# kevinh-e/BetaOne

Hardware: AMD Instinct MI355X
Metric: mcts_nodes_per_sec (higher is better)
Workload: dtype f32 (3 x f16 split, f32 accumulate)

## Files before the change

### betaone_amd/csrc/bo_engine.cpp

```cpp
#include "../../include/betaone_engine.h"
#include "../../include/betaone_lab.h"

#include "bo_tree.h"
#include "bo_fastw.h"
#include "bo_select_wide.h"
#include "bo_replay.h"
#include "bo_train.h"
#include "bo_metrics.h"
#include "bo_pgn.h"
#include "bo_san.h"
#include "bo_analyse.h"
#include "bo_reanalyse.h"
#include "bo_perft.h"
#include "bo_book.h"
#include "bo_merge.h"
#include "bo_tb.h"
#include "bo_nn_fused.h"
#include "bo_conv.h"
#include "bo_tower.h"
#include "bo_tower_wg.h"
#include "bo_tower_h.h"
#include "bo_tower_s.h"
#include "bo_tower_s16.h"
#include "bo_tower_h16.h"
#include "bo_heads.h"
#include "bo_tower_b1.h"
#include "bo_rt.h"
#include "bo_hostrng.h"

#include <math.h>
#include <stdio.h>
#include <string.h>
#include <string>
#include <vector>
#include <algorithm>
#include <deque>
#include <memory>
#include <type_traits>

static thread_local std::string g_err;
static int fail(int code, const std::string &msg) {
    g_err = msg;
    return code;
}
#define RT(call)                                                                                     \
    do {                                                                                             \
        int _rc = (call);                                                                            \
        if (_rc != 0) return fail(BO_E_HIP, std::string(#call) + ": " + rt_errstr(_rc));             \
    } while (0)

struct bo_engine {
    Eng d;
    FastW f;
    int fast_reuse = 1;
    int sel_profile = 0, sel_pending = 0;
    long long sel_launches = 0;
    double sel_ms = 0.0;
#if !defined(BO_WAVE_EMU)
    hipEvent_t sel_ev0 = nullptr, sel_ev1 = nullptr;
#endif
    bool fast = false;
    bo_config cfg;
    int device;
    std::vector<void *> allocs;
    int *d_go = nullptr, *d_action = nullptr;
    std::vector<int> h_i32;
    std::vector<HostRng> rng;
    int *d_res_blk = nullptr, *d_info_blk = nullptr;
    int *h_res = nullptr, *h_info = nullptr;
    int watch_seen = 0;
    double *h_noise = nullptr;
    int *h_go = nullptr;
    int *h_action = nullptr;
    int action_flip = 0;
    rt_event ev_action[2]{};
    bool ev_action_made[2] = {false, false};
    bool ship = true;
    bool prefetch_valid = false;
    std::vector<int> h_nl, h_term;
    bool nl_valid = false;
    void *setup_dev = nullptr, *setup_host = nullptr;
    size_t setup_cap = 0;
    std::vector<unsigned char> noise_pending;
    std::vector<int> lazy_want;
    bool begin_lazy = false, ev_begin_made = false;
    rt_event ev_begin{};
    double *h_turn_u = nullptr;
    int *h_turn_flags = nullptr;
    double *d_turn_pw = nullptr;
    std::vector<double> turn_pw_host;
    double turn_pw_tfinal = 0.0;
    int *d_turn_action = nullptr, *d_turn_state = nullptr, *d_turn_cres = nullptr;
    float *d_turn_rv = nullptr;
    int *d_turn_resigned = nullptr, *d_turn_rnext = nullptr;
    std::vector<int> resign_en;
    float resign_t = 0.0f;
    int resign_k = 1;
    float *d_root_value = nullptr;
    TbTable *d_tb_tabs = nullptr;
    std::vector<int> turn_want;
    bool turn_outstanding = false, ev_turn_made = false;
    rt_event ev_turn{};
    template <class T> int alloc(T **p, size_t n) {
        void *v = nullptr;
        int rc = rt_malloc(&v, n * sizeof(T));
        if (rc) return rc;
        allocs.push_back(v);
        *p = (T *)v;
        return 0;
    }
};

extern "C" int bo_abi_version(void) { return BO_ABI_VERSION; }
extern "C" const char *bo_last_error(void) { return g_err.c_str(); }

static const char *START_FEN = "rnbqkbnr/pppppppp/8/8/8/8/PPPPPPPP/RNBQKBNR w KQkq - 0 1";

static bool parse_fen(const char *fen, DPos *out) {
    memset(out, 0, sizeof(*out));
    const char *s = fen;
    while (*s == ' ') s++;
    int r = 7, f = 0;
    for (; *s && *s != ' '; s++) {
        char c = *s;
        if (c == '/') { r--; f = 0; continue; }
        if (c >= '1' && c <= '8') { f += c - '0'; continue; }
        int white = (c >= 'A' && c <= 'Z');
        char l = (char)(white ? c - 'A' + 'a' : c);
        int t = l == 'p' ? 0 : l == 'n' ? 1 : l == 'b' ? 2 : l == 'r' ? 3 : l == 'q' ? 4 : l == 'k' ? 5 : -1;
        if (t < 0 || r < 0 || f > 7) return false;
        out->bb[t] |= BIT(r * 8 + f);
        out->bb[white ? BB_WHITE : BB_BLACK] |= BIT(r * 8 + f);
        f++;
    }
    int turn = 1, ep = -1, half = 0, full = 1;
    uint32_t cr = 0;
    while (*s == ' ') s++;
    if (*s) { if (*s == 'w') turn = 1; else if (*s == 'b') turn = 0; else return false; s++; }
    while (*s == ' ') s++;
    for (; *s && *s != ' '; s++) {
        if (*s == 'K') cr |= 0x02u; else if (*s == 'Q') cr |= 0x04u; else if (*s == 'k') cr |= 0x08u;
        else if (*s == 'q') cr |= 0x10u; else if (*s != '-') return false;
    }
    const uint64_t wk = out->bb[BB_K] & out->bb[BB_WHITE] & BIT(4), bk = out->bb[BB_K] & out->bb[BB_BLACK] & BIT(60);
    const uint64_t wr = out->bb[BB_R] & out->bb[BB_WHITE], br = out->bb[BB_R] & out->bb[BB_BLACK];
    if (!wk || !(wr & BIT(7))) cr &= ~0x02u;
    if (!wk || !(wr & BIT(0))) cr &= ~0x04u;
    if (!bk || !(br & BIT(63))) cr &= ~0x08u;
    if (!bk || !(br & BIT(56))) cr &= ~0x10u;
    while (*s == ' ') s++;
    if (*s) {
        if (*s != '-') {
            if (s[0] < 'a' || s[0] > 'h' || s[1] < '1' || s[1] > '8') return false;
            ep = (s[1] - '1') * 8 + (s[0] - 'a');
            s += 2;
        } else s++;
    }
    while (*s == ' ') s++;
    if (*s) half = (int)strtol(s, (char **)&s, 10);
    while (*s == ' ') s++;
// ... 70 lines not shown
    c.nstride = c.NCAP;
    c.PLY_CAP = cfg->max_plies; c.TRK_CAP = cfg->max_plies;
    c.UL_MAX = fast ? 1 : c.B; c.CH_MAX = ch_max < 1 ? 1 : ch_max;
    c.cpuct = (float)cfg->cpuct;
    c.keep = (float)(1.0 - cfg->dirichlet_epsilon);
    c.eps = cfg->dirichlet_epsilon;
    c.use_noise = cfg->dirichlet_alpha > 0 ? 1 : 0;
    c.root_m = root_m;
    c.profile = 0;
    { const char *v = getenv("BETAONE_BURST_TWO_PATHS"); c.burst_two = (v && v[0] == '0') ? 0 : 1; }
    c.root_q = 0;
    const size_t G = (size_t)c.G, N = G * (size_t)c.NCAP;
    Eng &d = e->d;
    int rc = 0;
    float *sq = nullptr, *rcp = nullptr; int *wl = nullptr;
    rc |= e->alloc(&sq, (size_t)c.S + 2); rc |= e->alloc(&wl, (size_t)c.B + 1); rc |= e->alloc(&rcp, (size_t)c.S + 3);
    int **iscal[] = {&d.sims_done, &d.n_nodes, &d.rows, &d.n_runs, &d.n_ul, &d.req_nlegal, &d.status,
                     &d.trk_n, &d.n_hist, &d.ctx_mode, &d.root_nch, &d.stat_evals,
                     &d.stat_flushes, &d.stat_term_sims, &d.stat_levels, &d.stat_children_scanned, &e->d_go, &e->d_action};
    for (int **p : iscal) rc |= e->alloc(p, G);
    const size_t res_ints = G * (4 + 2 * (size_t)BO_RES_CAP) + 4, info_ints = G * 18;
    rc |= e->alloc(&e->d_res_blk, res_ints); rc |= e->alloc(&e->d_info_blk, info_ints);
    if (!rc) {
        d.res_n = e->d_res_blk; d.res_best_idx = e->d_res_blk + G; d.res_best_mv = e->d_res_blk + 2 * G; d.res_total = e->d_res_blk + 3 * G;
        d.res_idx = e->d_res_blk + 4 * G; d.res_val = reinterpret_cast<float *>(e->d_res_blk + 4 * G + G * BO_RES_CAP);
        d.res_watch = e->d_res_blk + G * (4 + 2 * (size_t)BO_RES_CAP); d.watch = nullptr; d.watch_n = 1;
        d.phase = e->d_info_blk; d.req_node = e->d_info_blk + G; d.root_nlegal = e->d_info_blk + 2 * G; d.root_term = e->d_info_blk + 3 * G;
        d.ply = e->d_info_blk + 4 * G;
        e->d_turn_action = e->d_info_blk + 5 * G; e->d_turn_state = e->d_info_blk + 6 * G; e->d_turn_cres = e->d_info_blk + 7 * G;
        e->d_turn_rv = reinterpret_cast<float *>(e->d_info_blk + 15 * G); e->d_turn_resigned = e->d_info_blk + 16 * G;
        e->d_turn_rnext = e->d_info_blk + 17 * G;
        rt_memset(e->d_res_blk, 0, res_ints * 4, nullptr); rt_memset(e->d_info_blk, 0, info_ints * 4, nullptr);
    }
    rc |= rt_host_alloc((void **)&e->h_res, res_ints * 4); rc |= rt_host_alloc((void **)&e->h_info, info_ints * 4);
    rc |= rt_host_alloc((void **)&e->h_noise, G * BO_MAX_MOVES * sizeof(double)); rc |= rt_host_alloc((void **)&e->h_go, G * 4);
    rc |= rt_host_alloc((void **)&e->h_action, 2 * G * 4);
    rc |= rt_host_alloc((void **)&e->h_turn_u, G * sizeof(double)); rc |= rt_host_alloc((void **)&e->h_turn_flags, G * 4);
    rc |= e->alloc(&e->d_turn_pw, (size_t)cfg->num_simulations + 1);
    { const char *v = getenv("BETAONE_TURN_COPIES"); e->ship = !(v && v[0] == '1'); }
    rc |= e->alloc(&d.gpos, G * c.PLY_CAP); rc |= e->alloc(&d.trk, G * c.TRK_CAP); rc |= e->alloc(&d.trk_cnt, G * c.TRK_CAP);
    rc |= e->alloc(&d.hist, G * 7);
    rc |= e->alloc(&d.n_visits, N); rc |= e->alloc(&d.parent, N); rc |= e->alloc(&d.first_child, N); rc |= e->alloc(&d.n_children, N);
    rc |= e->alloc(&d.q, N); rc |= e->alloc(&d.prior, N); rc |= e->alloc(&d.move, N); rc |= e->alloc(&d.term, N);
    rc |= e->alloc(&d.eval_slot, N); rc |= e->alloc(&d.npos, N);
    rc |= e->alloc(&d.run_leaf, G * c.B); rc |= e->alloc(&d.run_cnt, G * c.B);
    rc |= e->alloc(&d.ul_node, G * c.UL_MAX); rc |= e->alloc(&d.ul_nlegal, G * c.UL_MAX); rc |= e->alloc(&d.ul_value, G * c.UL_MAX);
    rc |= e->alloc(&d.ul_move, G * c.UL_MAX * BO_CH_CAP); rc |= e->alloc(&d.ul_prior, G * c.UL_MAX * BO_CH_CAP);
    rc |= e->alloc(&d.req_moves, G * BO_MAX_MOVES); rc |= e->alloc(&d.root_moves, G * BO_MAX_MOVES);
    rc |= e->alloc(&d.root_child_rank, G * 2 * BO_CH_CAP); rc |= e->alloc(&d.noise, G * BO_MAX_MOVES);
    rc |= e->alloc(&d.played, G * c.PLY_CAP);
    rc |= e->alloc(&d.prof, G * BO_PROF_SLOTS);
    rc |= e->alloc(&d.resign_cnt, 2 * G); rc |= e->alloc(&e->d_root_value, G);
    if (!rc) rt_memset(d.resign_cnt, 0, 2 * G * 4, nullptr);
    rc |= e->alloc(&e->d_tb_tabs, (size_t)TB_MAX_TABLES); rc |= e->alloc(&d.tb_stat, 3 * G);
    if (!rc) rt_memset(d.tb_stat, 0, 3 * G * 4, nullptr);
    d.tb_tabs = e->d_tb_tabs; d.tb_n = 0; d.tb_flags = 0;
    d.played_now = nullptr;
    if (fast) {
        FastW &f = e->f;
        const size_t L = (size_t)cfg->leaves_per_step;
        f.L = (int)L;
        f.sel_ut = 2; f.sel_flags = FW_SEL_OCT;
        const size_t expansions = (size_t)c.S + L + 2;
        f.NG = cfg->fast_arena_granules > 0 ? cfg->fast_arena_granules : (int)((6 * expansions + 8) * (32 / BO_FW_GR));
        if (f.NG < 64 || f.NG > BO_FW_LINK_MASK) { bo_engine_destroy(e); return fail(BO_E_ARG, "fast_arena_granules out of range (64 .. 2^24 - 1)"); }
        const size_t NR = (size_t)f.NG * BO_FW_GR;
        rc |= e->alloc(&f.arena, G * 2 * NR); rc |= e->alloc(&f.amove, G * 2 * NR);
        f.CS = (FWC_HEAD + FWR_FIELDS * (int)L + 31) / 32 * 32;
        rc |= e->alloc(&f.ctl, G * (size_t)f.CS);
        rc |= e->alloc(&f.played_now, G); rc |= e->alloc(&f.row_pos, G * L);
        rc |= e->alloc(&f.row_moves, G * L * BO_MAX_MOVES);
        rc |= e->alloc(&f.sim_path, G * L * BO_FW_PATH_CAP);
        float *st = nullptr, *rt = nullptr;
        rc |= e->alloc(&st, (size_t)BO_FW_SQRT_TAB); rc |= e->alloc(&rt, (size_t)BO_FW_RCP_TAB);
        if (!rc) {
            std::vector<float> hs2(BO_FW_SQRT_TAB), hr2(BO_FW_RCP_TAB, 0.0f);
            for (int n = 0; n < BO_FW_SQRT_TAB; n++) hs2[n] = (float)sqrt((double)n);
            for (int k = 1; k < BO_FW_RCP_TAB; k++) hr2[k] = (float)(1.0 / (double)k);
            rt_h2d(st, hs2.data(), hs2.size() * sizeof(float), nullptr); rt_h2d(rt, hr2.data(), hr2.size() * sizeof(float), nullptr);
            rt_sync(nullptr);
            f.sqrt_tab = st; f.rcp_tab = rt;
            rt_memset(f.ctl, 0, G * (size_t)f.CS * 4, nullptr);
            rt_memset(f.played_now, 0, G * 4, nullptr);
            d.played_now = f.played_now;
        }
    }
    if (rc) { bo_engine_destroy(e); return fail(BO_E_HIP, "device allocation failed"); }
    std::vector<float> hs((size_t)c.S + 2);
    for (int n = 0; n < c.S + 2; n++) hs[n] = (float)sqrt((double)n + 1e-8);
    std::vector<int> hw((size_t)c.B + 1);
    for (int k = 0; k <= c.B; k++) hw[k] = (int)(cfg->widen_coeff * sqrt((double)k));
    std::vector<float> hr((size_t)c.S + 3, 0.0f);
    for (int n = 1; n < c.S + 3; n++) hr[n] = (float)(1.0 / (double)n);
    rt_h2d(rcp, hr.data(), hr.size() * sizeof(float), nullptr);
    d.rcp_lut = rcp;
    rt_h2d(sq, hs.data(), hs.size() * sizeof(float), nullptr);
    rt_h2d(wl, hw.data(), hw.size() * sizeof(int), nullptr);
    d.sqrt_lut = sq; d.widen_lut = wl;
    for (int **p : iscal) rt_memset(*p, 0, G * sizeof(int), nullptr);
    rt_memset(d.noise, 0, G * BO_MAX_MOVES * sizeof(double), nullptr);
    rt_sync(nullptr);
    e->h_i32.resize(G);
    e->rng.resize(G);
    for (size_t g = 0; g < G; g++) hr_seed(&e->rng[g], (uint32_t)g);
    memset(e->h_noise, 0, G * BO_MAX_MOVES * sizeof(double));
    e->h_nl.resize(G); e->h_term.resize(G);
    *out = e;
// ... 149 lines not shown

extern "C" int bo_search_begin(bo_engine *e, const int32_t *go, const double *noise, float *nn_in_dev, void *stream) {
    return search_begin_impl(e, go, noise, false, nn_in_dev, stream);
}

static int launch_fw_select(bo_engine *e, const float *value_dev, int kind, void *stream) {
    const FastW &f = e->f;
    const int G = e->d.c.G, L = f.L;
    if (L == 4 && (f.sel_flags & FW_SEL_LANE)) {
        const int blocks = (G + 63) / 64;
        if (f.sel_flags & FW_SEL_NT) return RT_LAUNCH(bo_k_fw_select_lane_nt, blocks, stream, e->d, e->f, value_dev, kind);
        return RT_LAUNCH(bo_k_fw_select_lane, blocks, stream, e->d, e->f, value_dev, kind);
    }
    if (L <= 8 && (f.sel_flags & FW_SEL_QUAD)) {
        const int blocks = (G + 15) / 16;
#define SELQ(K) return RT_LAUNCH(K, blocks, stream, e->d, e->f, value_dev, kind)
        if (L > 4) SELQ(bo_k_fw_select_q4l8_0);
        if (f.sel_flags & FW_SEL_DENSE) SELQ(bo_k_fw_select_q4l4_4);
        if (f.sel_flags & FW_SEL_ROOT_IN_REGS) SELQ(bo_k_fw_select_q4l4_2);
        SELQ(bo_k_fw_select_q4l4_0);
#undef SELQ
    }
    if (L <= 8 && (f.sel_flags & FW_SEL_OCT)) {
        const int blocks = (G + 7) / 8;
        const int fl = f.sel_flags & 3;
#define SELO(K) return RT_LAUNCH(K, blocks, stream, e->d, e->f, value_dev, kind)
        if (L > 4) { if (fl & 2) SELO(bo_k_fw_select_o8l8_2); SELO(bo_k_fw_select_o8l8_0); }
        if (fl == 3) SELO(bo_k_fw_select_o8l4_3);
        if (fl == 2) SELO(bo_k_fw_select_o8l4_2);
        if (fl == 1) SELO(bo_k_fw_select_o8l4_1);
        SELO(bo_k_fw_select_o8l4_0);
#undef SELO
    }
    const int ut = L > 16 ? 1 : (L > 8 && f.sel_ut > 2) ? 2 : L > 4 ? (L > 8 ? 2 : 4) : f.sel_ut;
    const int grid = (G + 2 * ut - 1) / (2 * ut);
#define SEL(K) return RT_LAUNCH(K, grid, stream, e->d, e->f, value_dev, kind)
    const bool fancy = (f.sel_flags & FW_SEL_ROOT_IN_REGS) != 0;
    if (L > 16) { if (fancy) SEL(bo_k_fw_select_u1l64_3); SEL(bo_k_fw_select_u1l64_0); }
    if (L > 8) { if (fancy) SEL(bo_k_fw_select_u2l16_3); SEL(bo_k_fw_select_u2l16_0); }
    if (L > 4) { if (fancy) SEL(bo_k_fw_select_u4l8_3); SEL(bo_k_fw_select_u4l8_0); }
#define SEL8(UT)                                                                                  \
    switch (f.sel_flags & 7) {                                                                     \
        case 0: SEL(bo_k_fw_select_u##UT##l4_0); case 1: SEL(bo_k_fw_select_u##UT##l4_1);         \
        case 2: SEL(bo_k_fw_select_u##UT##l4_2); case 3: SEL(bo_k_fw_select_u##UT##l4_3);         \
        case 4: SEL(bo_k_fw_select_u##UT##l4_4); case 5: SEL(bo_k_fw_select_u##UT##l4_5);         \
        case 6: SEL(bo_k_fw_select_u##UT##l4_6); default: SEL(bo_k_fw_select_u##UT##l4_7);        \
    }
    if (ut >= 4) { SEL8(4) }
    SEL8(2)
#undef SEL8
#undef SEL
}

static int step_launch(bo_engine *e, const float *policy_dev, const float *value_dev, int policy_kind, float *nn_in_dev, void *stream, const StepTail &vt) {
    e->prefetch_valid = false;
    if (e->fast) {
        const int rows = e->d.c.G * e->f.L;
        if (policy_kind != BO_POLICY_NONE) RT(RT_LAUNCH(bo_k_fw_apply, rows, stream, e->d, e->f, policy_dev, policy_kind));
#if !defined(BO_WAVE_EMU)
        if (e->sel_profile) {
            if (!e->sel_ev0) { RT((int)hipEventCreate(&e->sel_ev0)); RT((int)hipEventCreate(&e->sel_ev1)); }
            if (e->sel_pending) {
                float ms = 0.0f;
                RT((int)hipEventSynchronize(e->sel_ev1));
                RT((int)hipEventElapsedTime(&ms, e->sel_ev0, e->sel_ev1));
                e->sel_ms += ms; e->sel_launches++; e->sel_pending = 0;
            }
            RT((int)hipEventRecord(e->sel_ev0, (hipStream_t)stream));
        }
#endif
        RT(launch_fw_select(e, value_dev, policy_kind, stream));
#if !defined(BO_WAVE_EMU)
        if (e->sel_profile) { RT((int)hipEventRecord(e->sel_ev1, (hipStream_t)stream)); e->sel_pending = 1; }
#endif
        RT(RT_LAUNCH(bo_k_fw_leaf, rows, stream, e->d, e->f, nn_in_dev));
    } else {
        if (e->d.tb_n > 0 && (e->d.tb_flags & TBF_SEARCH)) RT(RT_LAUNCH(bo_k_step_tb, e->d.c.G, stream, e->d, policy_dev, value_dev, policy_kind, nn_in_dev, vt));
        else RT(RT_LAUNCH(bo_k_step, e->d.c.G, stream, e->d, policy_dev, value_dev, policy_kind, nn_in_dev, vt));
    }
    return BO_OK;
}
extern "C" int bo_step(bo_engine *e, const float *policy_dev, const float *value_dev, int policy_kind, float *nn_in_dev,
                       void *stream) {
    if (!e || !nn_in_dev) return fail(BO_E_ARG, "null argument");
    if (policy_kind != BO_POLICY_NONE && (!policy_dev || !value_dev)) return fail(BO_E_ARG, "policy/value required");
    return step_launch(e, policy_dev, value_dev, policy_kind, nn_in_dev, stream, StepTail{nullptr, nullptr, nullptr, nullptr, 0});
}
extern "C" int bo_step_heads(bo_engine *e, const float *logits_dev, const float *vpart_dev, const float *b1_dev, const float *w2_dev,
                             const float *b2_dev, int rows, float *nn_in_dev, void *stream) {
    if (!e || !nn_in_dev || !logits_dev || !vpart_dev || !b1_dev || !w2_dev || !b2_dev) return fail(BO_E_ARG, "null argument");
    if (e->fast) return fail(BO_E_CONFIG, "bo_step_heads: the reference-semantics search only (fast mode evaluates rows, not games)");
    if (rows < e->d.c.G) return fail(BO_E_ARG, "bo_step_heads: the partial sums must hold a row per game (rows >= G)");
    return step_launch(e, logits_dev, nullptr, BO_POLICY_LOGITS, nn_in_dev, stream, StepTail{vpart_dev, b1_dev, w2_dev, b2_dev, rows});
}

extern "C" int bo_search_poll(bo_engine *e, int32_t *n_running, int32_t *n_requested, int32_t *requested_mask, void *stream) {
    if (!e) return fail(BO_E_ARG, "null engine");
    const size_t G = (size_t)e->d.c.G;
    RT(rt_d2h(e->h_info, e->d_info_blk, 2 * G * 4, stream));
    const int *ph = e->h_info, *rq = e->h_info + G;
    RT(rt_sync(stream));
    int run = 0, req = 0;
    for (size_t g = 0; g < G; g++) {
        bool r = ph[g] == PH_RUN;
        bool q = r && rq[g] >= 0;
        run += r; req += q;
        if (requested_mask) requested_mask[g] = q ? 1 : 0;
    }
    if (n_running) *n_running = run;
    if (n_requested) *n_requested = req;
    return BO_OK;
}

extern "C" int bo_search_stop(bo_engine *e, const int32_t *stop_mask, int32_t *sims_done, void *stream) {
    if (!e) return fail(BO_E_ARG, "null engine");
    if (e->fast) return fail(BO_E_CONFIG, "bo_search_stop: reference-semantics engines only");
    const size_t G = (size_t)e->d.c.G;
    const int *d_mask = nullptr;
    if (stop_mask) {
        memcpy(e->h_go, stop_mask, G * 4);
        RT(rt_h2d(e->d_go, e->h_go, G * 4, stream));
        d_mask = e->d_go;
    }
    RT(RT_LAUNCH(bo_k_stop, e->d.c.G, stream, e->d, d_mask));
    if (sims_done) RT(rt_d2h(sims_done, e->d.sims_done, G * 4, stream));
    RT(rt_sync(stream));
    return BO_OK;
}

extern "C" int bo_search_close(bo_engine *e, void *stream) {
    if (!e) return fail(BO_E_ARG, "null engine");
    if (e->fast) return fail(BO_E_CONFIG, "bo_search_close: reference-semantics engines only");
    if (e->d.c.root_q) return fail(BO_E_STATE, "bo_search_close: root values are on (a closed search's q values lack the last evaluation)");
    e->prefetch_valid = false;
    RT(RT_LAUNCH(bo_k_search_close, e->d.c.G, stream, e->d));
    return BO_OK;
}

static int ship(bo_engine *e, int *dst_a, const int *src_a, size_t n_a, int *dst_b, const int *src_b, size_t n_b, void *stream) {
    const size_t n = n_a > n_b ? n_a : n_b;
    const int blocks = (int)((n + 511) / 512 < 1 ? 1 : ((n + 511) / 512 > 128 ? 128 : (n + 511) / 512));
    RT(RT_LAUNCH(bo_k_ship, blocks, stream, dst_a, src_a, (int)n_a, dst_b, src_b, (int)n_b, blocks));
    (void)e;
    return BO_OK;
}

// ... 265 lines not shown
    const int G = e->d.c.G;
    const double alpha = e->cfg.dirichlet_alpha;
    if ((int)e->noise_pending.size() != G || alpha <= 0) return BO_OK;
    bool any = false;
    for (int g = 0; g < G; g++) any = any || e->noise_pending[g];
    if (!any) return BO_OK;
    host_pool().run(G, [&](int g) {
        if (e->noise_pending[g]) hr_dirichlet(&e->rng[g], alpha, e->h_nl[g], &e->h_noise[(size_t)g * BO_MAX_MOVES]);
    });
    e->nl_valid = true;
    int rc = upload_noise(e, e->noise_pending.data(), stream);
    e->nl_valid = false;
    std::fill(e->noise_pending.begin(), e->noise_pending.end(), 0);
    return rc;
}

extern "C" int bo_selfplay_turn(bo_engine *e, const int32_t *active, const int32_t *move_number, int32_t threshold, double t_initial,
                                double t_final, int32_t *res_n, int32_t *res_idx, float *res_val, int32_t *best_idx, int32_t *action_out,
                                const int32_t *want_next, float *nn_in_dev, int32_t *n_legal_out, int32_t *terminal_out, int32_t *go_out,
                                int32_t defer_noise, int32_t *completed, void *stream) {
    if (!e || !want_next || !nn_in_dev || !completed) return fail(BO_E_ARG, "null argument");
    *completed = 0;
    const bool poll_first = (defer_noise & 2) != 0, lazy_begin = (defer_noise & 4) != 0, prefetched = (defer_noise & 8) != 0;
    defer_noise &= 1;
    if (prefetched && !poll_first) return fail(BO_E_ARG, "bo_selfplay_turn: flag 8 (result block prefetched) goes with flag 2");
    if (lazy_begin && !defer_noise) return fail(BO_E_ARG, "bo_selfplay_turn: flag 4 (begin without waiting) needs flag 1 (noise later)");
    if (e->begin_lazy) return fail(BO_E_STATE, "bo_selfplay_begun has not collected the previous turn's roots yet");
    if (e->turn_outstanding) return fail(BO_E_STATE, "bo_selfplay_autoturn_collect has not collected the device's turn yet");
    int rc;
    if (poll_first) {
        const size_t G = (size_t)e->d.c.G;
        if (!(prefetched && e->prefetch_valid)) {
            rc = result_enqueue(e, stream, true);
            if (rc) return rc;
        }
        e->prefetch_valid = false;
        RT(rt_sync(stream));
        for (size_t g = 0; g < G; g++)
            if (e->h_info[g] == PH_RUN) { *completed = -1; return BO_OK; }
    }
    rc = selfplay_sample_impl(e, active, move_number, threshold, t_initial, t_final, res_n, res_idx, res_val, best_idx, action_out, poll_first, stream);
    if (rc) return rc;
    for (int g = 0; g < e->d.c.G; g++)
        if (action_out[g] == -3) return BO_OK;
    rc = bo_play(e, action_out, stream);
    if (rc) return rc;
    rc = lazy_begin ? selfplay_begin_lazy(e, want_next, nn_in_dev, stream)
                    : selfplay_begin_impl(e, want_next, nn_in_dev, n_legal_out, terminal_out, go_out, defer_noise != 0, stream);
    if (rc) return rc;
    *completed = lazy_begin ? 2 : 1;
    return BO_OK;
}

extern "C" int bo_selfplay_autoturn(bo_engine *e, const int32_t *active, const int32_t *move_number, int32_t threshold, double t_initial,
                                    double t_final, const int32_t *want_next, float *nn_in_dev, int32_t redo, void *stream) {
    if (!e || !active || !move_number || !want_next || !nn_in_dev) return fail(BO_E_ARG, "null argument");
    if (e->fast || e->d.c.root_m != 1 || e->d.c.S < 1)
        return fail(BO_E_CONFIG, "bo_selfplay_autoturn: reference-semantics engines whose root keeps <= 2 children (int(WIDEN_COEFF) == 1, NUM_SIMULATIONS >= 1)");
    if (!(fabs(t_initial - 1.0) < 1e-6) || t_final == 0.0 || !(t_final > 0.0))
        return fail(BO_E_CONFIG, "bo_selfplay_autoturn: TEMPERATURE_INITIAL must be 1 and TEMPERATURE_FINAL > 0 (other settings: bo_selfplay_turn)");
    if (!e->ship) return fail(BO_E_CONFIG, "bo_selfplay_autoturn is not available with BETAONE_TURN_COPIES=1");
    if (e->begin_lazy) return fail(BO_E_STATE, "bo_selfplay_begun has not collected the previous turn's roots yet");
    if (e->turn_outstanding) return fail(BO_E_STATE, "bo_selfplay_autoturn: the previous turn has not been collected");
    const int G = e->d.c.G, S = e->d.c.S;
    if (e->turn_pw_tfinal != t_final) {
        e->turn_pw_host.resize((size_t)S + 1);
        for (int c = 0; c <= S; c++) {
            const float p = (float)((double)c / (double)S);
            double x = pow((double)p, 1.0 / t_final);
            if (!isfinite(x)) x = 0.0;
            e->turn_pw_host[c] = x;
        }
        RT(rt_h2d(e->d_turn_pw, e->turn_pw_host.data(), ((size_t)S + 1) * sizeof(double), stream));
        RT(rt_sync(stream));
        e->turn_pw_tfinal = t_final;
    }
    if (!redo) {
        for (int g = 0; g < G; g++) {
            const double temp = move_number[g] < threshold ? t_initial : t_final;
            int fl = (active[g] ? 1 : 0) | (want_next[g] ? 4 : 0);
            if (active[g] && !(fabs(temp - 1.0) < 1e-6)) fl |= 2;
            if (active[g] && (int)e->resign_en.size() == G && e->resign_en[g]) fl |= 8;
            e->h_turn_flags[g] = fl;
            if (active[g]) e->h_turn_u[g] = hr_double(&e->rng[g]);
        }
        e->turn_want.assign(want_next, want_next + G);
    }
    TurnArgs a;
    a.u = e->h_turn_u; a.flags = e->h_turn_flags; a.pw = e->d_turn_pw;
    a.action = e->d_turn_action; a.state = e->d_turn_state; a.cres = e->d_turn_cres;
    a.root_value = e->d_turn_rv; a.resigned = e->d_turn_resigned; a.resign_next = e->d_turn_rnext;
    a.resign_t = e->resign_t; a.resign_k = e->resign_k;
    e->prefetch_valid = false;
    e->nl_valid = false;
    RT(RT_LAUNCH(bo_k_turn_sample, G, stream, e->d, a));
    RT(RT_LAUNCH(bo_k_turn_play, G, stream, e->d, a, nn_in_dev));
    const size_t Gs = (size_t)G, watch_off = Gs * (4 + 2 * (size_t)BO_RES_CAP);
    int rc = ship(e, e->h_info + 2 * Gs, (const int *)e->d_info_blk + 2 * Gs, 15 * Gs, e->h_res + watch_off, (const int *)e->d_res_blk + watch_off, 4, stream);
    if (rc) return rc;
    if (!e->ev_turn_made) { RT(rt_event_create(&e->ev_turn)); e->ev_turn_made = true; }
    RT(rt_event_record(e->ev_turn, stream));
    rc = bo_step(e, nullptr, nullptr, BO_POLICY_NONE, nn_in_dev, stream);
    if (rc) return rc;
    e->turn_outstanding = true;
    return BO_OK;
}

extern "C" int bo_selfplay_autoturn_ready(bo_engine *e, int32_t *ready_out) {
    if (!e || !ready_out) return fail(BO_E_ARG, "null argument");
    if (!e->turn_outstanding) return fail(BO_E_STATE, "no bo_selfplay_autoturn outstanding");
#if defined(BO_WAVE_EMU)
    *ready_out = 1;
#else
    const hipError_t q = hipEventQuery(e->ev_turn);
    if (q != hipSuccess && q != hipErrorNotReady) return fail(BO_E_HIP, std::string("hipEventQuery: ") + hipGetErrorString(q));
    *ready_out = q == hipSuccess ? 1 : 0;
#endif
    return BO_OK;
}

extern "C" int bo_selfplay_autoturn_collect_ex(bo_engine *e, int32_t *res_n, int32_t *res_idx, float *res_val, int32_t *best_idx,
                                               int32_t *action_out, int32_t *n_legal_out, int32_t *terminal_out, int32_t *go_out,
                                               float *root_value_out, int32_t *resigned_out, int32_t *completed) {
    if (!e || !res_n || !res_idx || !res_val || !action_out || !completed) return fail(BO_E_ARG, "null argument");
    if (!e->turn_outstanding) return fail(BO_E_STATE, "no bo_selfplay_autoturn outstanding");
    RT(rt_event_sync(e->ev_turn));
    e->turn_outstanding = false;
    *completed = 0;
    const int G = e->d.c.G;
    const size_t Gs = (size_t)G;
    const int *act = e->h_info + 5 * Gs, *st = e->h_info + 6 * Gs, *cres = e->h_info + 7 * Gs, *rsg = e->h_info + 16 * Gs;
    e->watch_seen |= e->h_res[Gs * (4 + 2 * (size_t)BO_RES_CAP)];
    bool running = false;
    for (int g = 0; g < G; g++) {
        if (st[g] == 2) return fail(BO_E_STATE, "bo_selfplay_autoturn: a search result the device sampler does not cover (slot " + std::to_string(g) + ")");
        running = running || st[g] == 1 || st[g] == 3;
    }
    if (running) { *completed = -1; return BO_OK; }
    const double alpha = e->cfg.dirichlet_alpha;
    if ((int)e->noise_pending.size() != G) e->noise_pending.assign(G, 0);
    for (int g = 0; g < G; g++) {
        const int *c = cres + (size_t)g * 8;
        action_out[g] = act[g];
        if (e->h_turn_flags[g] & 1) {
            res_n[g] = c[0];
            if (best_idx) best_idx[g] = c[1];
            res_idx[(size_t)g * BO_RES_CAP] = c[4]; res_idx[(size_t)g * BO_RES_CAP + 1] = c[5];
            memcpy(&res_val[(size_t)g * BO_RES_CAP], &c[6], 4); memcpy(&res_val[(size_t)g * BO_RES_CAP + 1], &c[7], 4);
        } else res_n[g] = 0;
        e->h_nl[g] = e->h_info[2 * Gs + g];
        e->h_term[g] = e->h_info[3 * Gs + g];
        const int go = e->turn_want[g] && e->h_term[g] == 0 && !rsg[g];
        e->h_go[g] = go;
        if (e->turn_want[g]) e->noise_pending[g] = 0;
        if (go && alpha > 0) e->noise_pending[g] = 1;
        if (n_legal_out) n_legal_out[g] = e->h_nl[g];
        if (terminal_out) terminal_out[g] = e->h_term[g];
        if (go_out) go_out[g] = go;
// ... 934 lines not shown
    if (!q_dev || !mix_dev || !loss5_dev) return fail(BO_E_ARG, "bo_train_loss_forward_mix: bad arguments");
    bool ok = false;
    train_dtype(logits_dtype, [&](auto *tl) {
        ok = train_dtype(value_dtype, [&](auto *tv) {
            BO_TRAIN_TYPES(tl, tv);
            rc = RT_LAUNCH((bo_k_loss_fwd_mix<TL, TV>), n, stream, (int)W, (const TL *)logits_dev, (const TV *)value_dev, (const int *)pi_idx_dev,
                           pi_val_dev, z_dev, q_dev, mix_dev, row_stats_dev);
        });
    });
    if (!ok) return fail(BO_E_CONFIG, "bo_train_loss_forward_mix: unsupported dtype");
    if (!rc) rc = RT_LAUNCH(bo_k_loss_reduce_mix, 1, stream, (int)n, (const float *)row_stats_dev, mix_dev, loss5_dev);
    if (rc) return fail(BO_E_HIP, std::string("bo_train_loss_forward_mix: ") + rt_errstr(rc));
    return BO_OK;
}

extern "C" int bo_train_loss_backward_mix(int32_t n, int32_t W, const void *logits_dev, int32_t logits_dtype, const void *value_dev,
                                          int32_t value_dtype, const int32_t *pi_idx_dev, const float *pi_val_dev, const float *z_dev,
                                          const float *q_dev, const float *mix_dev, const float *row_stats_dev, const float *grad_out_dev,
                                          void *dlogits_dev, void *dvalue_dev, void *stream) {
    int rc = train_loss_args("bo_train_loss_backward_mix", n, W, logits_dev, value_dev, pi_idx_dev, pi_val_dev, z_dev, row_stats_dev);
    if (rc) return rc;
    if (!q_dev || !mix_dev || !grad_out_dev || !dlogits_dev || !dvalue_dev) return fail(BO_E_ARG, "bo_train_loss_backward_mix: bad arguments");
    bool ok = false;
    train_dtype(logits_dtype, [&](auto *tl) {
        ok = train_dtype(value_dtype, [&](auto *tv) {
            BO_TRAIN_TYPES(tl, tv);
            rc = RT_LAUNCH((bo_k_loss_bwd_mix<TL, TV>), n, stream, (int)n, (int)W, (const TL *)logits_dev, (const TV *)value_dev,
                           (const int *)pi_idx_dev, pi_val_dev, z_dev, q_dev, mix_dev, row_stats_dev, grad_out_dev, (TL *)dlogits_dev,
                           (TV *)dvalue_dev);
        });
    });
    if (!ok) return fail(BO_E_CONFIG, "bo_train_loss_backward_mix: unsupported dtype");
    if (rc) return fail(BO_E_HIP, std::string("bo_train_loss_backward_mix: ") + rt_errstr(rc));
    return BO_OK;
}

extern "C" int bo_train_metrics(int32_t n, int32_t W, const void *logits_dev, int32_t logits_dtype, const void *value_dev, int32_t value_dtype,
                                const int32_t *pi_idx_dev, const float *pi_val_dev, const float *z_dev, const float *q_dev,
                                const int32_t *bucket_dev, int32_t n_buckets, float *rows_dev, double *accum_dev, void *stream) {
    int rc = train_loss_args("bo_train_metrics", n, W, logits_dev, value_dev, pi_idx_dev, pi_val_dev, z_dev, rows_dev);
    if (rc) return rc;
    if (n_buckets < 1 || !accum_dev) return fail(BO_E_ARG, "bo_train_metrics: bad arguments");
    bool ok = false;
    train_dtype(logits_dtype, [&](auto *tl) {
        ok = train_dtype(value_dtype, [&](auto *tv) {
            BO_TRAIN_TYPES(tl, tv);
            rc = RT_LAUNCH((bo_k_metrics_rows<TL, TV>), n, stream, (int)W, (const TL *)logits_dev, (const TV *)value_dev, (const int *)pi_idx_dev,
                           pi_val_dev, z_dev, q_dev, rows_dev);
        });
    });
    if (!ok) return fail(BO_E_CONFIG, "bo_train_metrics: unsupported dtype");
    if (!rc) rc = RT_LAUNCH(bo_k_metrics_reduce, n_buckets, stream, (int)n, (const float *)rows_dev, (const int *)bucket_dev, accum_dev);
    if (rc) return fail(BO_E_HIP, std::string("bo_train_metrics: ") + rt_errstr(rc));
    return BO_OK;
}

extern "C" int bo_debug_search_state(bo_engine *e, int32_t *out, void *stream) {
    if (!e || !out) return fail(BO_E_ARG, "bad arguments");
    if (e->fast) return fail(BO_E_CONFIG, "bo_debug_search_state: reference-semantics engines only");
    const size_t G = (size_t)e->d.c.G;
    const int *src[5] = {e->d.phase, e->d.sims_done, e->d.rows, e->d.req_node, e->d.n_nodes};
    for (int k = 0; k < 5; k++) RT(rt_d2h(out + k * G, src[k], G * 4, stream));
    RT(rt_sync(stream));
    return BO_OK;
}

extern "C" int bo_debug_tree(bo_engine *e, int slot, bo_node *out, int32_t cap, int32_t *n_nodes, void *stream) {
    if (!e || slot < 0 || slot >= e->d.c.G || !n_nodes) return fail(BO_E_ARG, "bad arguments");
    const EngCfg &c = e->d.c;
    int nn = 0;
    RT(rt_d2h(&nn, e->d.n_nodes + slot, 4, stream));
    RT(rt_sync(stream));
    if (e->fast) {
        const FastW &f = e->f;
        int head[FWC_HEAD];
        RT(rt_d2h(head, f.ctl + (size_t)slot * f.CS, sizeof(head), stream));
        RT(rt_sync(stream));
        const int cur = head[FWC_CUR], top = head[FWC_TOP];
        std::vector<WRec> A((size_t)top * BO_FW_GR);
        std::vector<bo_mv> M((size_t)top * BO_FW_GR);
        const size_t aoff = ((size_t)slot * 2 + (size_t)cur) * (size_t)f.NG * BO_FW_GR;
        RT(rt_d2h(A.data(), f.arena + aoff, A.size() * sizeof(WRec), stream));
        RT(rt_d2h(M.data(), f.amove + aoff, M.size() * sizeof(bo_mv), stream));
        RT(rt_sync(stream));
        std::vector<bo_node> nodes;
        std::vector<int> rec;
        auto push = [&](int r, int parent) {
            bo_node nd;
            nd.parent = parent; nd.n_visits = A[r].n; nd.first_child = 0; nd.n_children = 0; nd.q_value = A[r].w; nd.prior = A[r].prior;
            nd.move = r == 0 ? 0 : M[r];
            nd.terminal = A[r].link == FW_MATE ? 1 : A[r].link == FW_DRAW ? 2 : A[r].link >= 0 ? 0 : -1;
            nodes.push_back(nd); rec.push_back(r);
        };
        push(0, -1);
        for (size_t i = 0; i < nodes.size(); i++) {
            const int link = A[rec[i]].link;
            if (link < 0) continue;
            const int first = link & BO_FW_LINK_MASK, ng = ((link >> 24) & 127) + 1;
            if (first < 1 + BO_FW_HG || (size_t)(first + ng) * BO_FW_GR > A.size()) return fail(BO_E_HIP, "corrupt child-run link");
            nodes[i].first_child = (int)nodes.size();
            for (int k = 0; k < ng * BO_FW_GR; k++)
                if (A[(size_t)first * BO_FW_GR + k].n >= 0) { push(first * BO_FW_GR + k, (int)i); nodes[i].n_children++; }
        }
        *n_nodes = (int)nodes.size();
        if (!out) return BO_OK;
        if ((int)nodes.size() > cap) return fail(BO_E_ARG, "tree buffer too small");
// ... 1398 lines not shown
```

### betaone_amd/csrc/bo_tree.h

```cpp
#pragma once
#include "bo_chess.h"
#include "bo_tb_probe.h"
#include <math.h>

#define BO_CH_CAP 32
#define BO_PATH_CAP 1024
#define BO_RES_CAP 256
#define BO_PLANES 120
#ifndef BO_PROF_SLOTS
#define BO_PROF_SLOTS 16
#endif
#define BO_ROW (BO_PLANES * 64)

enum { PH_IDLE = 0, PH_RUN = 1, PH_DONE = 2 };
enum { ST_OK = 0, ST_NODE_OVERFLOW = 1, ST_DEPTH_OVERFLOW = 2, ST_NAN_SCORE = 4, ST_PLY_OVERFLOW = 8,
       ST_ILLEGAL_ACTION = 16, ST_UL_OVERFLOW = 32, ST_TRK_OVERFLOW = 64 };
enum { POLICY_NONE = 0, POLICY_LOGITS = 1, POLICY_PROBS = 2 };

struct EngCfg {
    int G, S, B;
    int NCAP, PLY_CAP, TRK_CAP;
    int nstride;
    int UL_MAX, CH_MAX;
    float cpuct, keep;
// ... 286 lines not shown
            }
            score = qv + u;
            if (!(score == score)) score = -__builtin_inff();
        }
        int bi = lane;
#define BO_SEL_STEP(os_expr, oi_expr)                                                   \
        {                                                                               \
            const float os = (os_expr);                                                 \
            const int oi = (oi_expr);                                                   \
            if (os > score || (os == score && oi < bi)) { score = os; bi = oi; }        \
        }
        BO_SEL_STEP(__builtin_bit_cast(float, BO_ROW_XCHG(__builtin_bit_cast(int, score), 0)), BO_ROW_XCHG(bi, 0))
        BO_SEL_STEP(__builtin_bit_cast(float, BO_ROW_XCHG(__builtin_bit_cast(int, score), 1)), BO_ROW_XCHG(bi, 1))
        BO_SEL_STEP(__builtin_bit_cast(float, BO_ROW_XCHG(__builtin_bit_cast(int, score), 2)), BO_ROW_XCHG(bi, 2))
        BO_SEL_STEP(__builtin_bit_cast(float, BO_ROW_XCHG(__builtin_bit_cast(int, score), 3)), BO_ROW_XCHG(bi, 3))
        if (nc > 16) {
            BO_SEL_STEP(bo_shfl_xor_f(score, 16), bo_shfl_xor(bi, 16))
            BO_SEL_STEP(bo_shfl_xor_f(score, 32), bo_shfl_xor(bi, 32))
        }
#undef BO_SEL_STEP
        score = __builtin_bit_cast(float, bo_readlane(__builtin_bit_cast(int, score), 0));
        bi = bo_readlane(bi, 0);
        if (!(score > -__builtin_inff())) { *flags |= ST_NAN_SCORE; bi = 0; }
        cur = fc + bi;
        levels++;
        if (lane == 0) path[levels] = cur;
        scanned += nc;
        pv = pv_next;
        pv_next = bo_readlane(n, bi);
        fc = bo_readlane(c_fc, bi);
        nc = bo_readlane(c_nc, bi);
        if (levels >= BO_PATH_CAP - 1) { *flags |= ST_DEPTH_OVERFLOW; break; }
    }
    if (lane == 0) { e.stat_levels[g] += levels; e.stat_children_scanned[g] += scanned; }
    *depth_out = levels;
    bo_sync();
    return cur;
}

#define BO_BURST_LEVELS 4
#define BO_BURST_FITS(S) (2 * (S) + 5 <= BO_NUM_ACTIONS)
BO_DEV_NOINLINE float bo_div_general(float x, float fn) { return x / fn; }
BO_DEV float bo_div_count(float x, float fn, float y) {
    const float q0 = x * y;
    const float r = __builtin_fmaf(-fn, q0, x);
    float q = __builtin_fmaf(r, y, q0);
    const float a = q0 < 0.0f ? -q0 : q0;
    if (x == 0.0f) q = q0;
    else if (!(a >= 1e-30f && a <= 1e30f)) q = bo_div_general(x, fn);
    return q;
}
template <bool TB>
BO_DEV int terminal_burst(const Eng &e, int g, const int *path, int d, float v, int sims_left, float *lds, bool *staged,
                          const int *pb = nullptr, int db = 0, float vb = 0.0f, int *n_swaps = nullptr) {
    const bool lone = TB && db < 0;
    const size_t no = NOFF(e, g);
    const int lane = bo_lane(), grp = lane >> 4, j = lane & 15;
    int c = 0;
    if (db > 0) {
        while (c <= d && c <= db && path[c] == pb[c]) c++;
        if (!(c >= 1 && c <= d - 1 && c <= db - 1)) db = 0;
    }
    bool two = db > 0;
    int nv[BO_BURST_LEVELS + 1];
    int fc[BO_BURST_LEVELS], ncs[BO_BURST_LEVELS], chosen[BO_BURST_LEVELS];
#pragma unroll
    for (int k = 0; k <= BO_BURST_LEVELS; k++) nv[k] = k <= d ? e.n_visits[no + path[k]] : 0;
#pragma unroll
    for (int k = 0; k < BO_BURST_LEVELS; k++) {
        fc[k] = k < d ? e.first_child[no + path[k]] : 0;
        ncs[k] = k < d ? e.n_children[no + path[k]] : 0;
        chosen[k] = k < d ? path[k + 1] - fc[k] : -1;
    }
    int my_fc = 0, my_nc = 0, my_chosen = -1;
    int b_fc = 0, b_nc = 0, b_chosen = -1;
    if (two && grp < db) { b_fc = e.first_child[no + pb[grp]]; b_nc = e.n_children[no + pb[grp]]; }
    int b_pv = (two && grp >= 1 && grp <= db) ? e.n_visits[no + pb[grp - 1]] : 0;
#pragma unroll
    for (int k = 0; k < BO_BURST_LEVELS; k++)
        if (grp == k) { my_fc = fc[k]; my_nc = ncs[k]; my_chosen = chosen[k]; }
    if (two && grp < db) b_chosen = pb[grp + 1] - b_fc;
    if (two && bo_ballot(grp < db && b_nc > 16) != 0) { two = false; db = 0; }
    bool have = grp < d && j < my_nc;
    const bool last = grp == d - 1;
    int cn = have ? e.n_visits[no + my_fc + j] : 0;
    float cq = have ? e.q[no + my_fc + j] : 0.0f;
    const float cp = have ? e.prior[no + my_fc + j] : 0.0f;
    int cterm = (have && last && e.n_children[no + my_fc + j] == 0) ? (int)e.term[no + my_fc + j] : -1;
    if (TB && (lone || cterm >= TERM_TB_WIN)) cterm = -1;
    int b_cn = 0, b_cterm = -1;
    float b_cq = 0.0f, b_cp = 0.0f;
    bool b_have = false;
    if (two) {
        b_have = grp >= c && grp < db && j < b_nc;
        b_cn = b_have ? e.n_visits[no + b_fc + j] : 0;
        b_cq = b_have ? e.q[no + b_fc + j] : 0.0f;
        b_cp = b_have ? e.prior[no + b_fc + j] : 0.0f;
        b_cterm = (b_have && grp == db - 1 && e.n_children[no + b_fc + j] == 0) ? (int)e.term[no + b_fc + j] : -1;
        if (TB && b_cterm >= TERM_TB_WIN) b_cterm = -1;
    }
    float v_cur = v, v_oth = vb;
    int d_oth = db;
    int done = 0;
    const int S = e.c.S;
    if (!*staged) {
        bo_sync();
        for (int t = lane; t < 2 * S + 5; t += 64) lds[t] = t < S + 2 ? e.sqrt_lut[t] : e.rcp_lut[t - (S + 2)];
// ... 44 lines not shown
        }
        const float cs = bo_shfl_f(score, (lane & 48) | (my_chosen & 15));
        const bool beat = have && (score > cs || (score == cs && j < my_chosen));
        const bool dead = grp < d && j == 0 && !(cs > -__builtin_inff());
        const uint64_t mb = bo_ballot(beat), md = bo_ballot(dead);
        if (md != 0) break;
        if ((mb & ~last_bits) != 0) {
            if (!two) break;
            const uint64_t upper = mb & ~last_bits;
            const int kb = (int)(__builtin_ctzll(upper) >> 4);
            if (kb != c - 1) break;
            int bi = j;
            float bs = score;
#define BO_BURST_STEP(kind)                                                                          \
            {                                                                                        \
                const float os = __builtin_bit_cast(float, BO_ROW_XCHG(__builtin_bit_cast(int, bs), kind)); \
                const int oi = BO_ROW_XCHG(bi, kind);                                                \
                if (os > bs || (os == bs && oi < bi)) { bs = os; bi = oi; }                          \
            }
            BO_BURST_STEP(0) BO_BURST_STEP(1) BO_BURST_STEP(2) BO_BURST_STEP(3)
#undef BO_BURST_STEP
            const int nb = bo_readlane(bi, 16 * (c - 1));
            const int ob = bo_readlane(b_chosen, 16 * (c - 1));
            if (nb != ob) break;
            float bscore = -__builtin_inff();
            if (b_have) {
                const float spb = BO_SQ(grp == c ? pv : b_pv);
                const float t2 = b_t1 * spb;
                float qv = 0.0f, u = t2;
                if (b_cn > 0) { qv = b_cq; u = bo_div_count(t2, (float)(1 + b_cn), b_y1); }
                bscore = qv + u;
                if (!(bscore == bscore)) bscore = -__builtin_inff();
            }
            const float bcs = bo_shfl_f(bscore, (lane & 48) | (b_chosen & 15));
            const bool bbeat = b_have && (bscore > bcs || (bscore == bcs && j < b_chosen));
            const bool bdead = grp >= c && grp < d_oth && j == 0 && !(bcs > -__builtin_inff());
            if (bo_ballot(bbeat) != 0 || bo_ballot(bdead) != 0) break;
            if (grp >= c) {
                { const int t_ = cn; cn = b_cn; b_cn = t_; }
                { const float t_ = cq; cq = b_cq; b_cq = t_; }
                { const float t_ = t1; t1 = b_t1; b_t1 = t_; }
                { const float t_ = y1; y1 = b_y1; b_y1 = t_; }
                { const bool t_ = have; have = b_have; b_have = t_; }
                { const int t_ = cterm; cterm = b_cterm; b_cterm = t_; }
                { const int t_ = my_fc; my_fc = b_fc; b_fc = t_; }
                { const int t_ = my_nc; my_nc = b_nc; b_nc = t_; }
            }
            if (grp > c) { const int t_ = pv; pv = b_pv; b_pv = t_; }
            if (grp >= c - 1) { const int t_ = my_chosen; my_chosen = b_chosen; b_chosen = t_; }
            { const int t_ = d; d = d_oth; d_oth = t_; }
            { const float t_ = v_cur; v_cur = v_oth; v_oth = t_; }
            last_l = grp == d - 1;
            last_bits = 0xFFFFull << (16 * (d - 1));
            if (n_swaps) *n_swaps += 1;
            continue;
        }
        if ((mb & last_bits) != 0) {
            int bi = j;
            float bs = score;
#define BO_BURST_STEP(kind)                                                                          \
            {                                                                                        \
                const float os = __builtin_bit_cast(float, BO_ROW_XCHG(__builtin_bit_cast(int, bs), kind)); \
                const int oi = BO_ROW_XCHG(bi, kind);                                                \
                if (os > bs || (os == bs && oi < bi)) { bs = os; bi = oi; }                          \
            }
            BO_BURST_STEP(0) BO_BURST_STEP(1) BO_BURST_STEP(2) BO_BURST_STEP(3)
#undef BO_BURST_STEP
            int bterm = (j == (bi & 15)) ? cterm : -2;
            { int o = BO_ROW_XCHG(bterm, 0); bterm = o > bterm ? o : bterm; }
            { int o = BO_ROW_XCHG(bterm, 1); bterm = o > bterm ? o : bterm; }
            { int o = BO_ROW_XCHG(bterm, 2); bterm = o > bterm ? o : bterm; }
            { int o = BO_ROW_XCHG(bterm, 3); bterm = o > bterm ? o : bterm; }
            const int src = 16 * (d - 1);
            const int nb = bo_readlane(bi, src), nt = bo_readlane(bterm, src);
            if (!(nt > 0)) break;
            if (last_l) my_chosen = nb;
            v_cur = nt == 1 ? 1.0f : 0.0f;
        }
    }
#undef BO_SQ
#undef BO_RC
    if (have) { e.n_visits[no + my_fc + j] = cn; e.q[no + my_fc + j] = cq; }
    if (two && b_have) { e.n_visits[no + b_fc + j] = b_cn; e.q[no + b_fc + j] = b_cq; }
    if (lane == 0) { e.n_visits[no] = nv[0]; if (root_q) e.q[no] = rq; }
    bo_sync();
    return done;
}

BO_DEV void backup_run(const Eng &e, int g, int leaf, float v, int cnt, int *scratch, int *flags, const int *known = nullptr,
                       int known_depth = -1) {
    const size_t no = NOFF(e, g);
    int d = 0;
    if (known_depth >= 0) {
        d = known_depth + 1;
    } else {
        for (int x = leaf; x >= 0 && d < BO_PATH_CAP; x = e.parent[no + x]) {
            if (bo_lane() == 0) scratch[d] = x;
            d++;
        }
        bo_sync();
    }
    for (int i = bo_lane(); i < d; i += 64) {
        const int nd = known_depth >= 0 ? known[known_depth - i] : scratch[i];
        const float val = (i & 1) ? -v : v;
        int n = e.n_visits[no + nd];
        float qv = e.q[no + nd];
        for (int c = 0; c < cnt; c++) {
// ... 149 lines not shown
    }
    for (int j = lane; j < n; j += 64) {
        int r = stable_rank(sh.pv, n, j);
        if (r < m) sh.rank_of[BO_CH_CAP + r] = j;
    }
    bo_sync();
    for (int r = 0; r < m; r++) {
        const int j = sh.rank_of[BO_CH_CAP + r];
        bool present = false;
        for (int k = 0; k < m; k++) present = present || sh.rank_of[k] == j;
        if (!present) {
            if (lane == 0) {
                init_node(e, no, 1 + nch, 0, sh.pv[j], mv[j], make_move(P, mv[j]));
                e.root_child_rank[(size_t)g * 2 * BO_CH_CAP + nch] = j;
            }
            nch++;
        }
    }
    if (lane == 0) { e.first_child[no] = 1; e.n_children[no] = nch; e.root_nch[g] = nch; }
    *n_nodes_io = 1 + nch;
    bo_sync();
}

struct StepTail { const float *vpart, *b1, *w2, *b2; int rows; };
struct TailRegs { float part[4][16], b1[4], w2[4], b2; };
BO_DEV void tail_load(const StepTail &t, int g, TailRegs &r) {
    const int lane = bo_lane();
    BO_UNROLL
    for (int w = 0; w < 4; w++) {
        BO_UNROLL
        for (int ks = 0; ks < 16; ks++) r.part[w][ks] = t.vpart[((size_t)ks * t.rows + g) * 256 + lane + 64 * w];
        r.b1[w] = t.b1[lane + 64 * w];
        r.w2[w] = t.w2[lane + 64 * w];
    }
    r.b2 = t.b2[0];
}
BO_DEV float tail_value(const TailRegs &r) {
    float s[4];
    BO_UNROLL
    for (int w = 0; w < 4; w++) {
        float h = 0.0f;
        BO_UNROLL
        for (int ks = 0; ks < 16; ks++) h += r.part[w][ks];
        h += r.b1[w];
        s[w] = (h > 0.0f ? h : 0.0f) * r.w2[w];
    }
    for (int m = 32; m >= 1; m >>= 1) {
        BO_UNROLL
        for (int w = 0; w < 4; w++) s[w] = s[w] + bo_shfl_xor_f(s[w], m);
    }
    return tanhf(((s[0] + s[1]) + (s[2] + s[3])) + r.b2);
}

BO_DEV void apply_leaf(const Eng &e, int g, int leaf, const float *row, int kind, const float *value_of, const StepTail &vt, StepShared &sh,
                       int *n_ul_io, int *flags) {
    const size_t no = NOFF(e, g);
    const int lane = bo_lane();
    const int n = e.req_nlegal[g];
    const bo_mv *mv = e.req_moves + (size_t)g * BO_MAX_MOVES;
    int slot = *n_ul_io;
    if (slot >= e.c.UL_MAX) { *flags |= ST_UL_OVERFLOW; slot = e.c.UL_MAX - 1; }
    const size_t uo = (size_t)g * e.c.UL_MAX + slot;
    float value;
    if (kind == POLICY_PROBS) {
        value = value_of[g];
        for (int j = lane; j < n; j += 64) sh.pv[j] = row[move_to_index(mv[j])];
    } else {
        float mx, sum;
        if (vt.vpart) {
            TailRegs tr;
            tail_load(vt, g, tr);
            row_max_sum(row, &mx, &sum);
            value = tail_value(tr);
        } else {
            value = value_of[g];
            row_max_sum(row, &mx, &sum);
        }
        for (int j = lane; j < n; j += 64) sh.pv[j] = bo_exp_row(row[move_to_index(mv[j])] - mx) / sum;
    }
    bo_sync();
    const int M = n < e.c.CH_MAX ? n : e.c.CH_MAX;
    for (int j = lane; j < n; j += 64) {
        int r = stable_rank(sh.pv, n, j);
        if (r < M) { e.ul_move[uo * BO_CH_CAP + r] = mv[j]; e.ul_prior[uo * BO_CH_CAP + r] = sh.pv[j]; }
    }
    if (lane == 0) {
        e.ul_node[uo] = leaf;
        e.ul_nlegal[uo] = n;
        e.ul_value[uo] = value;
        e.eval_slot[no + leaf] = (short)slot;
    }
    *n_ul_io = slot + 1;
    bo_sync();
}


BO_DEV float tb_leaf_value(int t, int kc) {
    const float m = 1.0f - (float)kc * (1.0f / 1024.0f);
    return t == TERM_TB_LOSS ? m : t == TERM_TB_WIN ? -m : 0.0f;
}
template <bool TB>
BO_DEV int step_body(const Eng &e, int g, const float *policy, const float *value, int kind, float *nn_in, StepShared &sh, const StepTail &vt) {
    const int lane = bo_lane();
    const size_t no = NOFF(e, g);
    int flags = 0;
    int sims = e.sims_done[g], rows = e.rows[g], n_runs = e.n_runs[g], n_ul = e.n_ul[g], n_nodes = e.n_nodes[g];
    int req = e.req_node[g];
    int *rl = e.run_leaf + (size_t)g * e.c.B, *rc = e.run_cnt + (size_t)g * e.c.B;
    float *row = nn_in + (size_t)g * BO_ROW;

    const bool prof = e.c.profile != 0;
    unsigned long long pc[8] = {0, 0, 0, 0, 0, 0, 0, 0};
    int n_iter = 0, n_first = 0, n_burst = 0, n_burst_sims = 0, n_general = 0, n_swaps = 0;
    unsigned long long tk = prof ? bo_clock() : 0ull;
    const unsigned long long t_start = tk;
#define BO_PROF(slot)                                                    \
    if (prof) { const unsigned long long _n = bo_clock(); pc[slot] += _n - tk; tk = _n; }
    if (req >= 0 && kind == POLICY_NONE) return n_nodes;
    const float *lut = e.sqrt_lut;
    if (req >= 0) {
        if (req == 0) apply_root(e, g, policy + (size_t)g * BO_NUM_ACTIONS, kind, sh, &n_nodes, &flags);
        else apply_leaf(e, g, req, policy + (size_t)g * BO_NUM_ACTIONS, kind, value, vt, sh, &n_ul, &flags);
        req = -1;
    }
    BO_PROF(0)
    int phase = PH_RUN;
    bool burst_tables_staged = false;
    int term_budget = e.c.B;
    int b_depth = 0;
    float b_tv = 0.0f;
    int path_leaf = -1, path_depth = -1;
    for (;;) {
        if (sims >= e.c.S) {
            if (rows > 0) { flush_pending(e, g, n_runs, n_ul, &n_nodes, sh.path2, &flags, path_leaf, sh.path, path_depth); rows = n_runs = n_ul = 0; }
            BO_PROF(5)
            phase = PH_DONE;
            break;
        }
        int depth;
        const int leaf = select_leaf(e, g, &flags, sh.path, &depth, lut);
        path_leaf = leaf; path_depth = depth;
        n_iter++;
        BO_PROF(1)
        int t = e.term[no + leaf];
        int tb_k = 0;
        if (TB && t >= TERM_TB_WIN) tb_k = (int)e.eval_slot[no + leaf];
        if (t < 0) {
            n_first++;
            const DPos P = e.npos[no + leaf];
            bool chk;
            const int n = bo_movegen(P, sh.moves, &chk);
            t = terminal_eval(e, g, sh.path, depth, P, sh.moves, n, chk, sh.moves2, sh.chain);
            if constexpr (TB) {
                const bool gate = t == 0 && leaf != 0 && (e.tb_flags & TBF_SEARCH) && bo_popc64(P.bb[BB_WHITE] | P.bb[BB_BLACK]) <= TB_MAX_MEN &&
                                  !(P.flags & F_CASTLE_MASK);
                if (bo_uniform(gate ? 1 : 0)) {
                    const uint32_t code = tb_lookup(e.tb_tabs, e.tb_n, P.bb, pos_turn(P));
                    const int k = (int)code - 2;
                    if (code == 1u) t = TERM_TB_DRAW;
                    else if (code >= 2u && code != TB_NO_TABLE && P.halfmove + k <= 100) t = (k & 1) ? TERM_TB_WIN : TERM_TB_LOSS;
                    if (t != 0) {
                        tb_k = t == TERM_TB_DRAW ? 0 : k < 512 ? k : 512;
                        if (lane == 0) { e.eval_slot[no + leaf] = (short)tb_k; e.tb_stat[3 * g] += 1; }
                    }
                }
            }
            if (lane == 0) e.term[no + leaf] = (signed char)t;
            if (t == 0) {
                for (int j = lane; j < n; j += 64) e.req_moves[(size_t)g * BO_MAX_MOVES + j] = sh.moves[j];
                if (lane == 0) e.req_nlegal[g] = n;
            }
            bo_sync();
            BO_PROF(2)
        }
        if (t > 0) {
            float tv = t == 1 ? 1.0f : 0.0f;
            const bool tb_leaf = TB && t >= TERM_TB_WIN;
            if (tb_leaf) tv = tb_leaf_value(t, tb_k);
            int applied = 1;
            bool small = depth <= BO_BURST_LEVELS && BO_BURST_FITS(e.c.S);
            for (int k = 0; k < depth && small; k++) small = e.n_children[no + sh.path[k]] <= 16;
            BO_PROF(6)
            const int may = e.c.S - sims < term_budget ? e.c.S - sims : term_budget;
            if (small) {
                const bool small_b = b_depth > 0 && e.c.burst_two != 0;
                applied = terminal_burst<TB>(e, g, sh.path, depth, tv, may, sh.probs, &burst_tables_staged, sh.bpath, tb_leaf ? -1 : small_b ? b_depth : 0, b_tv,
                                             &n_swaps);
                n_burst++; n_burst_sims += applied;
                bo_sync();
                if (lane <= depth) sh.bpath[lane] = sh.path[lane];
                b_depth = tb_leaf ? 0 : depth; b_tv = tv;
                bo_sync();
            }
            else { backup_run(e, g, leaf, tv, 1, sh.path2, &flags, sh.path, depth); n_general++; }
            BO_PROF(7)
            sims += applied;
            term_budget -= applied;
            if (lane == 0) e.stat_term_sims[g] += applied;
            if (tb_leaf && lane == 0) e.tb_stat[3 * g + 1] += applied;
            BO_PROF(3)
            if (term_budget <= 0 && sims < e.c.S) break;
            continue;
        }
        if (e.eval_slot[no + leaf] < 0) {
            encode_leaf(e, g, row, e.npos[no + leaf]);
            req = leaf;
            if (lane == 0) e.stat_evals[g] += 1;
            BO_PROF(4)
            break;
        }
        int cnt = e.c.B - rows;
        if (cnt > e.c.S - sims) cnt = e.c.S - sims;
        if (lane == 0) { rl[n_runs] = leaf; rc[n_runs] = cnt; }
        n_runs++;
        rows += cnt;
        sims += cnt;
        bo_sync();
        if (rows >= e.c.B) { flush_pending(e, g, n_runs, n_ul, &n_nodes, sh.path2, &flags, path_leaf, sh.path, path_depth); rows = n_runs = n_ul = 0; }
        BO_PROF(5)
    }
#undef BO_PROF
    if (prof && lane == 0) {
        const unsigned long long total = bo_clock() - t_start;
        if (e.c.profile == 1 || total > (unsigned long long)e.c.profile) {
            unsigned long long *pp = e.prof + (size_t)g * BO_PROF_SLOTS;
            pp[10] += (unsigned long long)n_burst; pp[11] += (unsigned long long)n_burst_sims; pp[12] += (unsigned long long)n_general;
            pp[13] += pc[6]; pp[14] += pc[7]; pp[15] += (unsigned long long)n_swaps;
            for (int i = 0; i < 6; i++) pp[i] += pc[i];
            pp[6] += total;
            pp[7] += 1;
            pp[8] += (unsigned long long)n_iter;
            pp[9] += (unsigned long long)n_first;
        }
    }
    if (lane == 0) {
        e.sims_done[g] = sims; e.rows[g] = rows; e.n_runs[g] = n_runs; e.n_ul[g] = n_ul; e.n_nodes[g] = n_nodes;
        e.req_node[g] = req; e.phase[g] = phase;
        if (flags) e.status[g] |= flags;
    }
    return n_nodes;
}
BO_KERNEL void bo_k_step(Eng e, const float *policy, const float *value, int kind, float *nn_in, StepTail vt) {
    BO_SHARED StepShared sh;
    const int g = bo_block();
    if (e.phase[g] != PH_RUN) return;
    step_body<false>(e, g, policy, value, kind, nn_in, sh, vt);
}
BO_KERNEL void bo_k_step_tb(Eng e, const float *policy, const float *value, int kind, float *nn_in, StepTail vt) {
    BO_SHARED StepShared sh;
    const int g = bo_block();
    if (e.phase[g] != PH_RUN) return;
    step_body<true>(e, g, policy, value, kind, nn_in, sh, vt);
}

BO_DEV int root_prepare(const Eng &e, int g, StepShared &sh) {
    const size_t no = NOFF(e, g);
    const int lane = bo_lane();
    const int ply = e.ply[g];
    const DPos P = e.gpos[(size_t)g * e.c.PLY_CAP + ply];
    if (lane == 0) {
        init_node(e, no, 0, -1, 1.0f, 0, P);
        e.n_nodes[g] = 1; e.sims_done[g] = 0; e.rows[g] = 0; e.n_runs[g] = 0; e.n_ul[g] = 0;
        e.req_node[g] = -1; e.phase[g] = PH_IDLE; e.root_nch[g] = 0;
        if (e.ctx_mode[g] == 0) {
            int nh = ply < 7 ? ply : 7;
            e.n_hist[g] = nh;
            for (int i = 0; i < nh; i++) e.hist[(size_t)g * 7 + i] = e.gpos[(size_t)g * e.c.PLY_CAP + ply - nh + i];
        }
    }
    bo_sync();
    bool chk;
    const int n = bo_movegen(P, sh.moves, &chk);
    if (lane == 0) sh.path[0] = 0;
    bo_sync();
    int t = terminal_eval(e, g, sh.path, 0, P, sh.moves, n, chk, sh.moves2, sh.chain);
    int adj = 0;
    if (bo_uniform(((e.tb_flags & TBF_ADJUDICATE) && t == 0 && bo_popc64(P.bb[BB_WHITE] | P.bb[BB_BLACK]) <= TB_MAX_MEN && !(P.flags & F_CASTLE_MASK)) ? 1 : 0)) {
        const uint32_t code = tb_lookup(e.tb_tabs, e.tb_n, P.bb, pos_turn(P));
        if (code == 1u) t = 2;
        else if (code >= 2u && code != TB_NO_TABLE && !((code - 2u) & 1u)) t = 3;
        adj = t != 0;
    }
    if (lane == 0) e.tb_stat[3 * g + 2] = adj;
    for (int j = lane; j < n; j += 64) {
        e.root_moves[(size_t)g * BO_MAX_MOVES + j] = sh.moves[j];
        e.req_moves[(size_t)g * BO_MAX_MOVES + j] = sh.moves[j];
    }
    if (lane == 0) { e.root_nlegal[g] = n; e.req_nlegal[g] = n; e.root_term[g] = t; e.term[no] = (signed char)t; }
    bo_sync();
    return t;
}

struct SetupArgs {
    const int *slots;
    const DPos *start;
    const bo_mv *moves;
    const int *n_moves;
    int max_moves;
    const DPos *hist;
    const int *n_hist;
    const DPos *trk;
    const int *trk_cnt;
    const int *n_trk;
    int max_trk;
};
// ... 22 lines not shown
            gp[ply + 1] = make_move(gp[ply], m);
            ply++;
        }
        e.ply[g] = ply;
        e.status[g] = st;
        e.ctx_mode[g] = explicit_ctx ? 1 : 0;
        if (explicit_ctx) {
            int nh = a.n_hist[i];
            e.n_hist[g] = nh;
            for (int k = 0; k < nh; k++) { DPos h = a.hist[(size_t)i * 7 + k]; finish_key(h); e.hist[(size_t)g * 7 + k] = h; }
            int nt = a.n_trk[i] < e.c.TRK_CAP ? a.n_trk[i] : e.c.TRK_CAP;
            for (int k = 0; k < nt; k++) { DPos t = a.trk[(size_t)i * a.max_trk + k]; finish_key(t); tk[k] = t; tc[k] = a.trk_cnt[(size_t)i * a.max_trk + k]; }
            e.trk_n[g] = nt;
        } else {
            for (int k = 0; k <= ply; k++) { tk[k] = gp[k]; tc[k] = 1; }
            e.trk_n[g] = ply + 1;
        }
        e.stat_evals[g] = e.stat_flushes[g] = e.stat_term_sims[g] = e.stat_levels[g] = e.stat_children_scanned[g] = 0;
        e.tb_stat[3 * g] = e.tb_stat[3 * g + 1] = 0;
        e.resign_cnt[2 * g] = e.resign_cnt[2 * g + 1] = 0;
    }
    bo_sync();
    root_prepare(e, g, sh);
}

BO_KERNEL void bo_k_search_begin(Eng e, const int *go, float *nn_in) {
    const int g = bo_block();
    if (!go[g]) return;
    encode_static(e, g, nn_in + (size_t)g * BO_ROW);
    if (bo_lane() == 0) e.phase[g] = PH_RUN;
}

BO_KERNEL void bo_k_search_begin_want(Eng e, const int *want, float *nn_in) {
    const int g = bo_block();
    if (!want[g] || e.root_term[g] != 0) return;
    encode_static(e, g, nn_in + (size_t)g * BO_ROW);
    if (bo_lane() == 0) e.phase[g] = PH_RUN;
}

BO_KERNEL void bo_k_stop(Eng e, const int *mask) {
    BO_SHARED int path[BO_PATH_CAP];
    const int g = bo_block(), lane = bo_lane();
    if ((mask && !mask[g]) || e.phase[g] != PH_RUN) return;
    int flags = 0, n_nodes = e.n_nodes[g];
    if (e.rows[g] > 0) flush_pending(e, g, e.n_runs[g], e.n_ul[g], &n_nodes, path, &flags);
    bo_sync();
    if (lane == 0) {
        e.rows[g] = 0; e.n_runs[g] = 0; e.n_ul[g] = 0; e.n_nodes[g] = n_nodes;
        e.req_node[g] = -1; e.phase[g] = PH_DONE;
        if (flags) e.status[g] |= flags;
    }
}

BO_KERNEL void bo_k_search_close(Eng e) {
    const int g = bo_block(), lane = bo_lane();
    if (e.phase[g] != PH_RUN) return;
    const size_t no = NOFF(e, g);
    const int req = e.req_node[g], n_nodes = e.n_nodes[g];
    const int cnt = e.c.S - e.sims_done[g];
    if (req <= 0 || req >= n_nodes || e.rows[g] != 0 || e.n_runs[g] != 0 || e.n_ul[g] != 0 || cnt < 1 || cnt > e.c.B) return;
    int c = e.widen_lut[cnt];
    const int nl = e.req_nlegal[g];
    if (c <= 0 || c > nl) c = nl;
    if (c > e.c.CH_MAX) c = e.c.CH_MAX;
    const int flags = n_nodes + c > e.c.NCAP ? ST_NODE_OVERFLOW : 0;
    int d = 0;
    for (int x = req; x >= 0 && x < n_nodes && d < BO_PATH_CAP; x = e.parent[no + x], d++)
        if (lane == 0) e.n_visits[no + x] += cnt;
    bo_sync();
    if (lane == 0) {
        e.sims_done[g] = e.c.S; e.rows[g] = 0; e.n_runs[g] = 0; e.n_ul[g] = 0;
        e.req_node[g] = -1; e.phase[g] = PH_DONE;
        if (flags) e.status[g] |= flags;
    }
}

BO_KERNEL void bo_k_ship(int *dst_a, const int *src_a, int n_a, int *dst_b, const int *src_b, int n_b, int n_blocks) {
    const int i0 = bo_block() * 64 + bo_lane(), stride = n_blocks * 64;
    for (int i = i0; i < n_a; i += stride) dst_a[i] = src_a[i];
    for (int i = i0; i < n_b; i += stride) dst_b[i] = src_b[i];
}

BO_DEV void result_body(const Eng &e, int g) {
    const int lane = bo_lane();
    if (g == 0 && lane == 0) e.res_watch[0] = e.watch ? (e.watch[0] | (e.watch_n > 1 && e.watch[1] ? 0x10000 : 0)) : 0;
    if (e.phase[g] != PH_DONE) return;
    const size_t no = NOFF(e, g);
    const int nch = e.n_children[no], fc = e.first_child[no], n = e.root_nlegal[g];
    const bo_mv *mv = e.root_moves + (size_t)g * BO_MAX_MOVES;
    int *ridx = e.res_idx + (size_t)g * BO_RES_CAP;
    float *rval = e.res_val + (size_t)g * BO_RES_CAP;
    const int v = lane < nch ? e.n_visits[no + fc + lane] : 0;
    const int total = bo_wave_sum(v);
    if (total > 0) {
        int key = lane < nch ? e.root_child_rank[(size_t)g * 2 * BO_CH_CAP + lane] : 0x7fffffff;
        int bv = v, bk = key;
        for (int m = 1; m < 64; m <<= 1) {
            int ov = bo_shfl_xor(bv, m), ok = bo_shfl_xor(bk, m);
            if (ov > bv || (ov == bv && ok < bk)) { bv = ov; bk = ok; }
        }
        const uint64_t nzmask = bo_ballot(lane < nch && v > 0);
        if (lane < nch && v > 0) {
            int o = bo_popc64(nzmask & (BIT(lane) - 1));
            ridx[o] = move_to_index(e.move[no + fc + lane]);
            rval[o] = (float)((double)v / (double)total);
        }
        if (lane == 0) {
            e.res_n[g] = bo_popc64(nzmask);
            e.res_best_mv[g] = mv[bk];
            e.res_best_idx[g] = move_to_index(mv[bk]);
            e.res_total[g] = total;
        }
    } else {
        for (int j = lane; j < n; j += 64) { ridx[j] = move_to_index(mv[j]); rval[j] = (float)(1.0 / (double)n); }
        if (lane == 0) {
            e.res_n[g] = n;
            e.res_best_mv[g] = n ? mv[0] : 0;
            e.res_best_idx[g] = n ? move_to_index(mv[0]) : -1;
            e.res_total[g] = 0;
        }
    }
}
BO_KERNEL void bo_k_result(Eng e) { result_body(e, bo_block()); }

BO_DEV int play_body(const Eng &e, int g, int a, StepShared &sh) {
    const int lane = bo_lane();
    if (a == -1) return -1;
    const int ply = e.ply[g], tn = e.trk_n[g];
// ... 26 lines not shown
        e.trk_cnt[(size_t)g * e.c.TRK_CAP + tn] = 1;
        e.trk_n[g] = tn + 1;
    }
    bo_sync();
    return root_prepare(e, g, sh);
}
BO_KERNEL void bo_k_play(Eng e, const int *action) {
    BO_SHARED StepShared sh;
    play_body(e, bo_block(), action[bo_block()], sh);
}

struct TurnArgs {
    const double *u;
    const int *flags;
    const double *pw;
    int *action;
    int *state;
    int *cres;
    float *root_value;
    int *resigned;
    int *resign_next;
    float resign_t;
    int resign_k;
};

BO_DEV int turn_sample(int n, int i0, int c0, int i1, int c1, int total, int S, bool power, const double *pw, double u, bool *ok) {
    *ok = true;
    if (n < 1 || n > 2 || total < 1) { *ok = false; return -1; }
    float p0 = (float)((double)c0 / (double)total), p1 = n == 2 ? (float)((double)c1 / (double)total) : 0.0f;
    if (n == 2 && i1 < i0) { int t = i0; i0 = i1; i1 = t; float q = p0; p0 = p1; p1 = q; t = c0; c0 = c1; c1 = t; }
    if (power) {
        if (total != S) { *ok = false; return -1; }
        double s0 = pw[c0], s1 = n == 2 ? pw[c1] : 0.0;
        const double sum = s0 + s1;
        if (!(sum > 1e-9)) { *ok = false; return -1; }
        p0 = (float)(s0 / sum);
        p1 = (float)(s1 / sum);
        const float rs = p0 + p1;
        if (__builtin_fabsf(rs - 1.0f) > (float)1e-6 && rs > (float)1e-9) { p0 = p0 / rs; p1 = p1 / rs; }
    }
    const float prob_sum = p0 + p1;
    if (__builtin_fabsf(prob_sum - 1.0f) > (float)1e-6) {
        if (prob_sum > (float)1e-9) { p0 = p0 / prob_sum; p1 = p1 / prob_sum; }
        else { *ok = false; return -1; }
    }
    const double d0 = (double)p0, d1 = (double)p1;
    if (__builtin_fabs((d0 + d1) - 1.0) > 3.4e-4 || d0 < 0 || d1 < 0) { *ok = false; return -1; }
    const double k0 = d0, k1 = d0 + d1;
    const double last = n == 2 ? k1 : k0;
    if (n == 1) return i0;
    return (k0 / last > u) ? i0 : i1;
}

BO_KERNEL void bo_k_turn_sample(Eng e, TurnArgs a) {
    const int g = bo_block(), lane = bo_lane();
    result_body(e, g);
    const int fl = a.flags[g], ph = e.phase[g];
    int st = 0, act = -1, n = 0, ia = -1, ib = -1, ca = 0, cb = 0, total = 0, rsg = 0, rnext = -1;
    float rv = 0.0f;
    if (e.watch && (e.watch[0] != 0 || (e.watch_n > 1 && e.watch[1] != 0))) st = 3;
    else if (ph == PH_RUN) st = 1;
    else if ((fl & 1) && ph == PH_DONE) {
        const size_t no = NOFF(e, g);
        const int nch = e.n_children[no], fc = e.first_child[no];
        const int v = lane < nch ? e.n_visits[no + fc + lane] : 0;
        const int idx = lane < nch ? move_to_index(e.move[no + fc + lane]) : -1;
        total = bo_wave_sum(v);
        const uint64_t nz = bo_ballot(v > 0);
        n = bo_popc64(nz);
        if (n >= 1) { const int l0 = bo_lsb64(nz); ia = bo_shfl(idx, l0); ca = bo_shfl(v, l0); }
        if (n >= 2) { const int l1 = bo_lsb64(nz & (nz - 1)); ib = bo_shfl(idx, l1); cb = bo_shfl(v, l1); }
        bool ok;
        act = turn_sample(n, ia, ca, ib, cb, total, e.c.S, (fl & 2) != 0, a.pw, a.u[g], &ok);
        if (!ok) { st = 2; act = -1; }
        rv = e.q[no];
        if (fl & 8) {
            const int cnt = e.resign_cnt[2 * g + (e.ply[g] & 1)];
            rnext = rv < a.resign_t ? cnt + 1 : 0;
            if (st == 0 && rnext >= a.resign_k) { rsg = 1; act = -1; }
        }
    }
    if (lane == 0) {
        a.root_value[g] = rv; a.resigned[g] = rsg; a.resign_next[g] = rnext;
        a.action[g] = act; a.state[g] = st;
        int *c = a.cres + (size_t)g * 8;
        c[0] = n; c[1] = e.res_best_idx[g]; c[2] = e.res_best_mv[g]; c[3] = total; c[4] = ia; c[5] = ib;
        c[6] = n >= 1 ? __builtin_bit_cast(int, (float)((double)ca / (double)total)) : 0;
        c[7] = n >= 2 ? __builtin_bit_cast(int, (float)((double)cb / (double)total)) : 0;
    }
}

BO_KERNEL void bo_k_turn_play(Eng e, TurnArgs a, float *nn_in) {
    BO_SHARED StepShared sh;
    const int g = bo_block(), lane = bo_lane();
    bool bad = false;
    for (int j0 = 0; j0 < e.c.G; j0 += 64) bad = bad || bo_ballot(j0 + lane < e.c.G && a.state[j0 + lane] != 0) != 0;
    if (bad) return;
    if (lane == 0 && a.resign_next[g] >= 0) e.resign_cnt[2 * g + (e.ply[g] & 1)] = a.resign_next[g];
    if (a.resigned[g]) return;
    int t = play_body(e, g, a.action[g], sh);
    if (t < 0) t = e.root_term[g];
    if (!(a.flags[g] & 4) || t != 0) return;
    encode_static(e, g, nn_in + (size_t)g * BO_ROW);
    if (lane == 0) e.phase[g] = PH_RUN;
}

BO_KERNEL void bo_k_root_value(Eng e, float *out) {
    const int g = bo_block() * 64 + bo_lane();
    if (g < e.c.G) out[g] = e.q[NOFF(e, g)];
}

BO_KERNEL void bo_k_encode_game(Eng e, int g, int first, float *out) {
    const int i = first + bo_block(), s = bo_lane();
    const DPos *gp = e.gpos + (size_t)g * e.c.PLY_CAP;
    float *row = out + (size_t)bo_block() * BO_ROW;
    const int h0 = i - 7 > 0 ? i - 7 : 0, nb = i + 1 - h0;
    for (int pl = 0; pl < (8 - nb) * 14; pl++) row[pl * 64 + s] = 0.0f;
    for (int k = 0; k < nb; k++) {
        DPos H = gp[h0 + k];
        encode_block(row, 8 - nb + k, H, tracker_reps(e, g, H));
    }
    encode_scalars(row, gp[i]);
}

BO_KERNEL void bo_k_encode_positions(const DPos *pos, int n_pos, int first, float *out) {
    const int i = first + bo_block(), s = bo_lane();
    float *row = out + (size_t)bo_block() * BO_ROW;
    const int h0 = i - 7 > 0 ? i - 7 : 0, nb = i + 1 - h0;
    for (int pl = 0; pl < (8 - nb) * 14; pl++) row[pl * 64 + s] = 0.0f;
    for (int k = 0; k < nb; k++) {
        const DPos H = pos[h0 + k];
        int c = 0;
        for (int j = s; j < n_pos; j += 64) c += key_equal(pos[j], H) ? 1 : 0;
        c = bo_wave_sum(c);
        encode_block(row, 8 - nb + k, H, c > 1 ? c - 1 : 0);
    }
    encode_scalars(row, pos[i]);
}

BO_KERNEL void bo_k_movegen(const DPos *pos, bo_mv *out, int *n_out, int *check_out) {
    BO_SHARED bo_mv mv[BO_MAX_MOVES];
    const int i = bo_block(), lane = bo_lane();
    DPos P = pos[i];
    bool chk;
    const int n = bo_movegen(P, mv, &chk);
    for (int j = lane; j < n; j += 64) out[(size_t)i * BO_MAX_MOVES + j] = mv[j];
    if (lane == 0) { n_out[i] = n; check_out[i] = chk ? 1 : 0; }
}
```

### betaone_amd/engine.py

```python
from __future__ import annotations

import ctypes as C
import os
from typing import Dict, List, Optional, Sequence, Tuple

import numpy as np
import torch

NUM_ACTIONS = 4672
INPUT_CHANNELS = 120
ROW_FLOATS = 120 * 64
MAX_LEGAL = 256
RES_CAP = 256
POLICY_NONE, POLICY_LOGITS, POLICY_PROBS = 0, 1, 2

STATUS_BITS = {1: "node overflow", 2: "depth overflow", 4: "NaN PUCT score", 8: "ply overflow",
               16: "illegal action", 32: "leaf cache overflow", 64: "tracker overflow", 128: "position range outside the array",
               256: "pi wider than the record's rows"}
ST_PLY_OVERFLOW, ST_ILLEGAL_ACTION = 8, 16
ST_PI_OVERFLOW = 256
ST_NODE_OVERFLOW = 1


LAZY_BEGIN = "lazy-begin"
# ... 31 lines not shown

class BoAnalysis(C.Structure):
    _fields_ = [("terminal", C.c_int32), ("n_legal", C.c_int32), ("total_visits", C.c_int32), ("best_move", C.c_int32),
                ("root_value", C.c_float), ("played_is_child", C.c_int32), ("played_visits", C.c_int32), ("played_q", C.c_float),
                ("pv_len", C.c_int32), ("pv", C.c_int32 * PV_CAP), ("phase", C.c_int32), ("status", C.c_int32), ("ply", C.c_int32),
                ("sims_done", C.c_int32), ("watch", C.c_int32), ("reserved", C.c_int32 * 2)]


ANALYSIS_DTYPE = np.dtype([("terminal", "<i4"), ("n_legal", "<i4"), ("total_visits", "<i4"), ("best_move", "<i4"), ("root_value", "<f4"),
                           ("played_is_child", "<i4"), ("played_visits", "<i4"), ("played_q", "<f4"), ("pv_len", "<i4"),
                           ("pv", "<i4", (PV_CAP,)), ("phase", "<i4"), ("status", "<i4"), ("ply", "<i4"), ("sims_done", "<i4"),
                           ("watch", "<i4"), ("reserved", "<i4", (2,))])
REANALYSIS_DTYPE = np.dtype([("terminal", "<i4"), ("n_legal", "<i4"), ("total_visits", "<i4"), ("best_idx", "<i4"), ("root_value", "<f4"),
                             ("pi_n", "<i4"), ("played_prob", "<f4"), ("has_old", "<i4"), ("agree", "<i4"), ("tv", "<f4"), ("phase", "<i4"),
                             ("status", "<i4"), ("ply", "<i4"), ("sims_done", "<i4"), ("watch", "<i4"), ("reserved", "<i4")])
PH_IDLE, PH_RUN, PH_DONE = 0, 1, 2


class BoHeadWeights(C.Structure):
    _fields_ = [("wp", C.c_void_p), ("bp", C.c_void_p), ("w1", C.c_void_p), ("b1", C.c_void_p), ("w2", C.c_void_p), ("b2", C.c_void_p)]


_I32P = C.POINTER(C.c_int32)
_F32P = C.POINTER(C.c_float)
_F64P = C.POINTER(C.c_double)

_SYMBOLS = {
    "bo_abi_version": (C.c_int, []),
    "bo_last_error": (C.c_char_p, []),
    "bo_engine_create": (C.c_int, [C.POINTER(BoConfig), C.c_int, C.POINTER(C.c_void_p)]),
    "bo_engine_destroy": (None, [C.c_void_p]),
    "bo_games_reset": (C.c_int, [C.c_void_p, C.c_int, _I32P, C.POINTER(C.c_char_p), C.POINTER(C.c_char_p), C.c_void_p]),
    "bo_games_reset_ex": (C.c_int, [C.c_void_p, C.c_int, _I32P, C.POINTER(C.c_char_p), C.POINTER(C.c_char_p),
                                    C.POINTER(BoPosition), _I32P, C.POINTER(BoPosition), _I32P, _I32P, C.c_void_p]),
    "bo_root_info": (C.c_int, [C.c_void_p, _I32P, _I32P, _I32P, C.c_void_p]),
    "bo_search_begin": (C.c_int, [C.c_void_p, _I32P, _F64P, C.c_void_p, C.c_void_p]),
    "bo_step": (C.c_int, [C.c_void_p, C.c_void_p, C.c_void_p, C.c_int, C.c_void_p, C.c_void_p]),
    "bo_step_heads": (C.c_int, [C.c_void_p] * 6 + [C.c_int, C.c_void_p, C.c_void_p]),
    "bo_search_poll": (C.c_int, [C.c_void_p, _I32P, _I32P, _I32P, C.c_void_p]),
    "bo_search_stop": (C.c_int, [C.c_void_p, _I32P, _I32P, C.c_void_p]),
    "bo_search_close": (C.c_int, [C.c_void_p, C.c_void_p]),
    "bo_search_result": (C.c_int, [C.c_void_p, _I32P, _I32P, _F32P, _I32P, _I32P, _I32P, C.c_void_p]),
    "bo_play": (C.c_int, [C.c_void_p, _I32P, C.c_void_p]),
    "bo_game_export": (C.c_int, [C.c_void_p, C.c_int, C.POINTER(BoPosition), _I32P, C.c_int32, _I32P, C.c_void_p]),
    "bo_game_encode": (C.c_int, [C.c_void_p, C.c_int, C.c_int, C.c_int, C.c_void_p, C.c_void_p]),
    "bo_rng_seed": (C.c_int, [C.c_void_p, C.c_int, C.c_uint32]),
    "bo_rng_state": (C.c_int, [C.c_void_p, C.c_int, C.c_int, C.POINTER(C.c_uint32), _I32P, _I32P, _F64P]),
    "bo_selfplay_sample": (C.c_int, [C.c_void_p, _I32P, _I32P, C.c_int32, C.c_double, C.c_double, _I32P, _I32P, _F32P,
                                     _I32P, _I32P, C.c_void_p]),
    "bo_selfplay_turn": (C.c_int, [C.c_void_p, _I32P, _I32P, C.c_int32, C.c_double, C.c_double, _I32P, _I32P, _F32P, _I32P, _I32P, _I32P,
                                   C.c_void_p, _I32P, _I32P, _I32P, C.c_int32, _I32P, C.c_void_p]),
    "bo_selfplay_noise": (C.c_int, [C.c_void_p, C.c_void_p]),
    "bo_selfplay_autoturn": (C.c_int, [C.c_void_p, _I32P, _I32P, C.c_int32, C.c_double, C.c_double, _I32P, C.c_void_p, C.c_int32, C.c_void_p]),
    "bo_selfplay_autoturn_ready": (C.c_int, [C.c_void_p, _I32P]),
    "bo_selfplay_autoturn_collect": (C.c_int, [C.c_void_p, _I32P, _I32P, _F32P, _I32P, _I32P, _I32P, _I32P, _I32P, _I32P]),
    "bo_selfplay_autoturn_collect_ex": (C.c_int, [C.c_void_p, _I32P, _I32P, _F32P, _I32P, _I32P, _I32P, _I32P, _I32P, _F32P, _I32P, _I32P]),
    "bo_engine_root_values": (C.c_int, [C.c_void_p, C.c_int32]),
    "bo_selfplay_resign": (C.c_int, [C.c_void_p, _I32P, C.c_float, C.c_int32]),
    "bo_search_root_value": (C.c_int, [C.c_void_p, _F32P, C.c_void_p]),
    "bo_pgn_movetext_text": (C.c_int, [C.c_int32, C.c_void_p, C.c_void_p, C.c_int32, C.c_int32, C.c_char_p, _I32P, C.c_char_p, C.c_char_p,
                                       C.c_char_p, C.c_int64, C.POINTER(C.c_int64)]),
    "bo_search_result_prefetch": (C.c_int, [C.c_void_p, C.c_void_p]),
    "bo_selfplay_begun": (C.c_int, [C.c_void_p, _I32P, _I32P, _I32P]),
    "bo_selfplay_begin": (C.c_int, [C.c_void_p, _I32P, C.c_void_p, _I32P, _I32P, _I32P, C.c_void_p]),
    "bo_records_encode": (C.c_int, [C.c_int, C.POINTER(BoPosition), C.c_int, C.c_int, C.c_void_p, C.c_void_p]),
    "bo_fast_options": (C.c_int, [C.c_void_p, C.c_int32, C.c_int32, C.c_int32]),
    "bo_nn_tower_status": (C.c_int, [C.c_void_p, _I32P, C.c_void_p]),
    "bo_nn_tower_word": (C.c_int, [C.c_void_p, C.POINTER(C.c_void_p)]),
    "bo_replay_create": (C.c_int, [C.c_int64, C.c_int, C.c_int, C.POINTER(C.c_void_p)]),
    "bo_replay_add_game": (C.c_int, [C.c_void_p, C.c_int32, C.POINTER(BoPosition), C.c_int32, _I32P, _I32P, _F32P, _F32P, C.POINTER(C.c_int64), C.c_void_p]),
    "bo_replay_size": (C.c_int, [C.c_void_p, C.POINTER(C.c_int64), C.POINTER(C.c_int64)]),
    "bo_replay_sample": (C.c_int, [C.c_void_p, C.c_int32, C.POINTER(C.c_int64), C.c_void_p, C.c_void_p, C.c_void_p, C.c_void_p]),
    "bo_replay_sample_sparse": (C.c_int, [C.c_void_p, C.c_int32, C.POINTER(C.c_int64)] + [C.c_void_p] * 5),
    "bo_replay_add_game_values": (C.c_int, [C.c_void_p, C.c_int32, C.POINTER(BoPosition), C.c_int32, _I32P, _I32P, _F32P, _F32P, _F32P,
                                            C.POINTER(C.c_int64), C.c_void_p]),
    "bo_replay_values": (C.c_int, [C.c_void_p, C.POINTER(C.c_int64)]),
    "bo_replay_sample_sparse_q": (C.c_int, [C.c_void_p, C.c_int32, C.POINTER(C.c_int64)] + [C.c_void_p] * 6),
    "bo_replay_destroy": (None, [C.c_void_p]),
    "bo_replay_merge_create": (C.c_int, [C.c_void_p, C.c_int64, C.POINTER(C.c_int64), C.c_int32, C.POINTER(C.c_void_p)]),
    "bo_replay_merge_create_ex": (C.c_int, [C.c_void_p, C.c_int64, C.POINTER(C.c_int64), C.c_int32, C.c_int64, C.c_void_p, C.POINTER(C.c_void_p)]),
    "bo_replay_merge_info": (C.c_int, [C.c_void_p, C.c_void_p]),
    "bo_replay_merge_groups": (C.c_int, [C.c_void_p, C.POINTER(C.c_int64), _I32P]),
    "bo_replay_sample_merged": (C.c_int, [C.c_void_p, C.c_void_p, C.c_int32, C.POINTER(C.c_int64)] + [C.c_void_p] * 6),
    "bo_replay_merge_destroy": (None, [C.c_void_p]),
    "bo_replay_sample_sym": (C.c_int, [C.c_void_p, C.c_int32, C.POINTER(C.c_int64), _I32P] + [C.c_void_p] * 5),
    "bo_replay_sample_sparse_sym": (C.c_int, [C.c_void_p, C.c_int32, C.POINTER(C.c_int64), _I32P] + [C.c_void_p] * 6),
    "bo_replay_sample_sparse_q_sym": (C.c_int, [C.c_void_p, C.c_int32, C.POINTER(C.c_int64), _I32P] + [C.c_void_p] * 7),
    "bo_replay_sample_merged_sym": (C.c_int, [C.c_void_p, C.c_void_p, C.c_int32, C.POINTER(C.c_int64), _I32P] + [C.c_void_p] * 7),
    "bo_nn_b1_create": (C.c_int, [C.c_void_p, C.c_int, C.c_int, C.c_int, C.c_int, C.POINTER(C.c_void_p)]),
    "bo_nn_b1_forward": (C.c_int, [C.c_void_p, C.c_void_p, C.c_void_p, C.c_int, C.c_void_p]),
    "bo_nn_b1_status": (C.c_int, [C.c_void_p, _I32P, C.c_void_p]),
    "bo_nn_b1_destroy": (None, [C.c_void_p]),
    "bo_engine_watch": (C.c_int, [C.c_void_p, C.c_void_p]),
    "bo_engine_watch_words": (C.c_int, [C.c_void_p, C.c_void_p, C.c_int32]),
    "bo_nn_b1_word": (C.c_int, [C.c_void_p, C.POINTER(C.c_void_p)]),
    "bo_engine_watch_seen": (C.c_int, [C.c_void_p, _I32P, C.c_int32]),
    "bo_engine_status": (C.c_int, [C.c_void_p, _I32P, _I32P, _I32P, _I32P, _I32P, _I32P, C.c_void_p]),
    "bo_movegen_batch": (C.c_int, [C.c_void_p, C.c_int, C.POINTER(BoPosition), _I32P, _I32P, _I32P, C.c_void_p]),
    "bo_nn_bias_act": (C.c_int, [C.c_void_p, C.c_void_p, C.c_void_p, C.c_int, C.c_int, C.c_void_p]),
    "bo_nn_se_residual": (C.c_int, [C.c_void_p, C.c_void_p, C.c_void_p, C.c_void_p, C.c_void_p, C.c_int, C.c_int, C.c_int,
                                    C.c_void_p]),
    "bo_nn_se_residual_small": (C.c_int, [C.c_void_p, C.c_void_p, C.c_void_p, C.c_void_p, C.c_void_p, C.c_int, C.c_int, C.c_int,
                                          C.c_void_p]),
    "bo_nn_heads": (C.c_int, [C.c_void_p] * 11 + [C.c_int, C.c_int, C.c_void_p]),
    "bo_nn_heads_f16": (C.c_int, [C.c_void_p] * 11 + [C.c_int, C.c_int, C.c_void_p]),
    "bo_nn_conv3x3": (C.c_int, [C.c_void_p, C.c_void_p, C.c_void_p, C.c_void_p, C.c_void_p, C.c_int, C.c_int, C.c_int, C.c_int,
# ... 4 lines not shown
                                     C.c_int, C.POINTER(C.c_void_p)]),
    "bo_nn_tower_forward": (C.c_int, [C.c_void_p, C.c_void_p, C.c_void_p, C.c_void_p, C.c_void_p, C.c_int, C.c_void_p]),
    "bo_device_wall_clock_khz": (C.c_int, [C.c_int, _I32P]),
    "bo_stream_create_cu_mask": (C.c_int, [C.c_int, C.POINTER(C.c_uint32), C.c_int, C.POINTER(C.c_void_p)]),
    "bo_stream_destroy": (C.c_int, [C.c_void_p]),
    "bo_nn_value_tail": (C.c_int, [C.c_void_p, C.c_void_p, C.c_void_p, C.c_void_p, C.c_int, C.c_int, C.c_void_p]),
    "bo_nn_tower_destroy": (None, [C.c_void_p]),
    "bo_nn_tower_pair_check": (C.c_int, [C.c_void_p, C.c_void_p]),
    "bo_nn_tower_forward_pair": (C.c_int, [C.c_void_p] * 6 + [C.c_int, C.c_void_p]),
    "bo_nn_heads_pair": (C.c_int, [C.c_void_p, C.c_void_p, C.POINTER(BoHeadWeights), C.POINTER(BoHeadWeights)] + [C.c_void_p] * 4
                         + [C.c_int, C.c_int, C.c_void_p]),
    "bo_nn_merge_rows": (C.c_int, [C.c_void_p] * 7 + [C.c_int, C.c_int, C.c_void_p]),
    "bo_match_select": (C.c_int, [C.c_void_p] * 4),
    "bo_train_loss_forward": (C.c_int, [C.c_int32, C.c_int32, C.c_void_p, C.c_int32, C.c_void_p, C.c_int32] + [C.c_void_p] * 6),
    "bo_train_loss_backward": (C.c_int, [C.c_int32, C.c_int32, C.c_void_p, C.c_int32, C.c_void_p, C.c_int32] + [C.c_void_p] * 8),
    "bo_train_loss_forward_mix": (C.c_int, [C.c_int32, C.c_int32, C.c_void_p, C.c_int32, C.c_void_p, C.c_int32] + [C.c_void_p] * 8),
    "bo_train_loss_backward_mix": (C.c_int, [C.c_int32, C.c_int32, C.c_void_p, C.c_int32, C.c_void_p, C.c_int32] + [C.c_void_p] * 10),
    "bo_train_metrics": (C.c_int, [C.c_int32, C.c_int32, C.c_void_p, C.c_int32, C.c_void_p, C.c_int32] + [C.c_void_p] * 5
                         + [C.c_int32, C.c_void_p, C.c_void_p, C.c_void_p]),
    "bo_pgn_parse": (C.c_int, [C.c_void_p, C.c_int64, C.c_int32, C.c_int64, C.c_int64, C.POINTER(C.c_int64), C.POINTER(C.c_void_p)]),
    "bo_pgn_size": (C.c_int, [C.c_void_p] + [C.POINTER(C.c_int64)] * 3),
    "bo_pgn_export": (C.c_int, [C.c_void_p, _I32P, _I32P, C.c_void_p, C.c_void_p, _I32P, _F32P]),
    "bo_pgn_replay": (C.c_int, [C.c_void_p, C.POINTER(C.c_int64), C.c_int64, C.c_void_p, C.c_int64] + [C.c_void_p] * 4 + [_I32P, _I32P, C.c_void_p]),
    "bo_pgn_sample": (C.c_int, [C.c_void_p, C.c_void_p, C.c_void_p, C.c_int32] + [C.c_void_p] * 7),
    "bo_pgn_destroy": (None, [C.c_void_p]),
    "bo_san_render": (C.c_int, [C.c_int32, C.c_int32] + [C.c_void_p] * 7),
    "bo_position_fen": (C.c_int, [C.POINTER(BoPosition), C.c_char_p, C.c_int32]),
    "bo_games_reset_dev": (C.c_int, [C.c_void_p, C.c_int, C.c_void_p, C.c_void_p, C.c_int64, C.c_void_p, C.c_void_p, C.c_void_p]),
    "bo_search_begin_dev": (C.c_int, [C.c_void_p] * 4),
    "bo_analysis_result": (C.c_int, [C.c_void_p] * 4),
    "bo_records_ring": (C.c_int, [C.c_void_p, C.c_int64, C.c_void_p, C.c_void_p]),
    "bo_reanalysis_result": (C.c_int, [C.c_void_p] * 6 + [C.c_int32] + [C.c_void_p] * 4),
    "bo_book_insert": (C.c_int, [C.c_void_p, C.c_int64, C.c_int64] + [C.c_void_p] * 5 + [C.c_int64] + [C.c_void_p] * 11 + [C.c_uint32, C.c_void_p]),
    "bo_pgn_after": (C.c_int, [C.c_void_p, C.c_void_p, C.c_int64, C.c_int32] + [C.c_void_p] * 4),
    "bo_pgn_spans": (C.c_int, [C.c_void_p, C.POINTER(C.c_int64), C.POINTER(C.c_int64)]),
    "bo_pgn_movetext": (C.c_int, [C.c_int32, C.c_void_p, C.c_void_p, C.c_int32, C.c_int32, C.c_void_p, C.c_char_p, C.c_char_p, C.c_int64,
                                  C.POINTER(C.c_int64)]),
    "bo_perft": (C.c_int, [C.c_int, C.c_int32, C.POINTER(C.c_char_p), C.c_int32, C.c_int64, C.c_uint32, C.c_void_p, C.c_void_p, C.c_void_p,
                           C.POINTER(C.c_int64), C.c_void_p]),
    "bo_tb_create": (C.c_int, [C.c_int, C.c_char_p, C.POINTER(C.c_void_p), C.c_int32, C.POINTER(C.c_void_p)]),
    "bo_tb_build": (C.c_int, [C.c_void_p, C.c_int32, _I32P, C.c_void_p]),
    "bo_tb_verify": (C.c_int, [C.c_void_p, C.POINTER(C.c_uint64), C.c_void_p]),
    "bo_tb_stats": (C.c_int, [C.c_void_p, C.c_void_p]),
    "bo_tb_download": (C.c_int, [C.c_void_p, C.c_void_p, C.c_int64]),
    "bo_tb_upload": (C.c_int, [C.c_void_p, C.c_void_p, C.c_int64, C.c_int32]),
    "bo_tb_probe": (C.c_int, [C.POINTER(C.c_void_p), C.c_int32, C.c_void_p, C.c_int32, C.c_void_p, C.c_void_p, C.c_void_p]),
    "bo_engine_tablebases": (C.c_int, [C.c_void_p, C.POINTER(C.c_void_p), C.c_int32, C.c_int32]),
    "bo_engine_tb_stats": (C.c_int, [C.c_void_p, _I32P, _I32P, _I32P, C.c_void_p]),
    "bo_tb_destroy": (None, [C.c_void_p]),
}
_LAB_SYMBOLS = {
    "bo_debug_tree": (C.c_int, [C.c_void_p, C.c_int, C.POINTER(BoNode), C.c_int32, _I32P, C.c_void_p]),
    "bo_debug_search_state": (C.c_int, [C.c_void_p, _I32P, C.c_void_p]),
    "bo_debug_fast": (C.c_int, [C.c_void_p, C.c_int, _I32P, C.c_int32, _I32P, C.c_void_p]),
    "bo_event_pair_overhead": (C.c_int, [_F64P, C.c_int32, C.c_void_p]),
    "bo_nn_b1_profile": (C.c_int, [C.c_void_p, C.c_int, C.POINTER(C.c_uint64), C.c_int]),
    "bo_fast_stats": (C.c_int, [C.c_void_p, C.POINTER(C.c_uint64), C.POINTER(C.c_uint64), _I32P, C.c_int32, _F64P, C.POINTER(C.c_int64),
                               C.c_void_p]),
    "bo_debug_profile": (C.c_int, [C.c_void_p, C.c_int, C.POINTER(C.c_uint64), C.c_void_p]),
    "bo_debug_stamp": (C.c_int, [C.c_void_p, C.c_uint64, C.c_uint64, C.c_void_p]),
    "bo_nn_tower_forward_timed": (C.c_int, [C.c_void_p, C.c_void_p, C.c_void_p, C.c_void_p, C.c_void_p, C.c_int, C.c_void_p, C.c_void_p]),
    "bo_select_wide": (C.c_int, [C.c_void_p, C.c_void_p, C.c_void_p, C.c_void_p, C.c_int, C.c_int, C.c_float, C.c_int,
                                 C.c_void_p, C.c_void_p, C.c_void_p]),
}

HIP_LIB_PATH = os.path.join(os.path.dirname(os.path.abspath(__file__)), "csrc", "libbetaone_hip.so")


def bind(cdll: C.CDLL) -> C.CDLL:
    for name, (res, args) in list(_SYMBOLS.items()) + list(_LAB_SYMBOLS.items()):
        fn = getattr(cdll, name)
        fn.restype = res
        fn.argtypes = args
    return cdll


_hip_lib: Optional[C.CDLL] = None
ABI_VERSION = 18
PROF_SLOTS = 16
METRIC_ROW = {name: k for k, name in enumerate((
    "BAD", "HAS_POLICY", "DECISIVE", "RANK", "TOP1", "TOP3", "TOP5", "ARGMAX_IN_SUPPORT", "CE", "TARGET_ENTROPY", "NET_ENTROPY", "P_TOP",
    "P_SUPPORT", "SE_Z", "SE_Q", "ABS_V", "SIGN_OK", "Z", "V"))}
METRIC = {name: k for k, name in enumerate((
    "N_ROWS", "N_BAD", "N_POLICY_ROWS", "N_DECISIVE", "SUM_RANK", "SUM_TOP1", "SUM_TOP3", "SUM_TOP5", "SUM_ARGMAX_IN_SUPPORT", "SUM_CE",
    "SUM_TARGET_ENTROPY", "SUM_NET_ENTROPY", "SUM_P_TOP", "SUM_P_SUPPORT", "SUM_SE_Z", "SUM_SE_Q", "SUM_ABS_V", "SUM_SIGN_OK", "SUM_Z", "SUM_V"))}
METRIC_ROW_COLS, METRIC_COLS = len(METRIC_ROW), len(METRIC)


def load_hip_library() -> C.CDLL:
    global _hip_lib
    if _hip_lib is None:
        from . import build as _build

        if not os.path.exists(HIP_LIB_PATH):
            raise EngineError(f"{HIP_LIB_PATH} is missing: build it with `python -m betaone_amd.build` "
                              "(hipcc --offload-arch=gfx950); betaone_amd has no CPU fallback")
        if _build.needs_build():
            raise EngineError(f"{HIP_LIB_PATH} was not built from the sources next to it (csrc/*.h changed since): "
                              "run `python -m betaone_amd.build`")
        _hip_lib = bind(C.CDLL(HIP_LIB_PATH))
        if _hip_lib.bo_abi_version() != ABI_VERSION:
            raise EngineError(f"libbetaone_hip.so ABI version {_hip_lib.bo_abi_version()} != {ABI_VERSION} (include/betaone_engine.h)")
    return _hip_lib


def runtime_device(requested) -> torch.device:
    dev = torch.device(requested)
    if dev.type != "cuda":
        raise EngineError(f"betaone_amd runs on an MI355X (device 'cuda' / 'cuda:N', got {requested!r}); there is no CPU path")
    return torch.device("cuda", dev.index if dev.index is not None else torch.cuda.current_device())


def cu_partition_masks(n_cu: int, parts: int, layout: str = "contiguous") -> list:
    if parts < 1 or n_cu < parts:
        raise ValueError(f"cannot split {n_cu} CUs into {parts} parts")
    per, words = n_cu // parts, (n_cu + 31) // 32
    out = []
    for p in range(parts):
        m = np.zeros(words, dtype=np.uint32)
        idx = (np.arange(p * per, (p + 1) * per) if layout == "contiguous" else np.arange(n_cu) if layout == "full"
               else np.arange(per) * parts + p)
        np.bitwise_or.at(m, idx // 32, (np.uint32(1) << (idx % 32).astype(np.uint32)))
        out.append(m)
    return out


class MaskedStream:

    def __init__(self, device: torch.device, mask_words: np.ndarray):
        self.lib = load_hip_library()
        self.mask = np.ascontiguousarray(mask_words, dtype=np.uint32)
# ... 11 lines not shown
            self.handle = None


def move_to_uci(m: int) -> str:
    f, t, p = m & 63, (m >> 6) & 63, (m >> 12) & 7
    s = "abcdefgh"[f & 7] + str((f >> 3) + 1) + "abcdefgh"[t & 7] + str((t >> 3) + 1)
    return s + (" pnbrqk"[p] if p else "")


def _i32(a) -> np.ndarray:
    return np.ascontiguousarray(a, dtype=np.int32)


def _p(a: np.ndarray, typ=_I32P):
    return a.ctypes.data_as(typ)


class PositionList:

    def __init__(self, raw, n: int):
        self.raw, self.n = raw, n

    def __len__(self) -> int:
        return self.n

    def __getitem__(self, i):
        if isinstance(i, slice):
            return [self.raw[k] for k in range(*i.indices(self.n))]
        if i < 0:
            i += self.n
        if not 0 <= i < self.n:
            raise IndexError(i)
        return self.raw[i]

    def __iter__(self):
        return (self.raw[k] for k in range(self.n))


class Engine:

    def __init__(self, n_games: int, num_simulations: int = 250, mcts_batch_size: int = 96, cpuct: float = 1.0,
                 widen_coeff: float = 1.5, dirichlet_alpha: float = 0.1, dirichlet_epsilon: float = 0.25,
                 max_plies: int = 1024, device: int = 0, fast: bool = False, leaves_per_step: int = 8, fast_arena_granules: int = 0):
        self.lib = load_hip_library()
        self.G = int(n_games)
        self.fast, self.L = bool(fast), int(leaves_per_step) if fast else 1
        self.cfg = BoConfig(n_games, num_simulations, mcts_batch_size, max_plies, cpuct, widen_coeff, dirichlet_alpha,
                            dirichlet_epsilon, 1 if fast else 0, self.L, int(fast_arena_granules))
        self.rows = self.G * self.L
        self.num_simulations, self.dirichlet_alpha = num_simulations, dirichlet_alpha
        h = C.c_void_p()
        self._check(self.lib.bo_engine_create(C.byref(self.cfg), device, C.byref(h)))
        self.h = h

    def close(self):
        if getattr(self, "h", None):
            self.lib.bo_engine_destroy(self.h)
            self.h = None

    def __del__(self):
        try:
            self.close()
        except Exception:
            pass

    def _check(self, rc: int):
        if rc != 0:
            raise EngineError(f"betaone engine error {rc}: {self.lib.bo_last_error().decode()}")

    @staticmethod
    def _strs(items: Optional[Sequence[Optional[str]]], n: int):
        arr = (C.c_char_p * n)()
        for i in range(n):
            v = items[i] if items is not None else None
            arr[i] = v.encode() if v is not None else None
        return arr

    def reset(self, slots: Sequence[int], fens: Optional[Sequence[Optional[str]]] = None,
              moves: Optional[Sequence[Optional[str]]] = None, stream: int = 0):
        s = _i32(slots)
        n = len(s)
        self._check(self.lib.bo_games_reset(self.h, n, _p(s), self._strs(fens, n), self._strs(moves, n), stream))

    def reset_ex(self, slots, fens, moves, hist: Sequence[Sequence[BoPosition]],
                 trk: Sequence[Sequence[Tuple[BoPosition, int]]], stream: int = 0):
        s = _i32(slots)
        n = len(s)
        harr = (BoPosition * (7 * n))()
        nh = np.zeros(n, dtype=np.int32)
        off = np.zeros(n + 1, dtype=np.int32)
        flat, cnts = [], []
        for i in range(n):
            nh[i] = len(hist[i])
            for k, p in enumerate(hist[i]):
                harr[i * 7 + k] = p
            for p, c in trk[i]:
                flat.append(p)
                cnts.append(c)
            off[i + 1] = len(flat)
        tarr = (BoPosition * max(1, len(flat)))(*flat)
        tc = _i32(cnts if cnts else [0])
        self._check(self.lib.bo_games_reset_ex(self.h, n, _p(s), self._strs(fens, n), self._strs(moves, n), harr, _p(nh),
                                               tarr, _p(tc), _p(off), stream))

    def reset_dev(self, n: int, slots_ptr: int, pos_ptr: int, capacity: int, first_ptr: int, ply_ptr: int, stream: int = 0):
        self._check(self.lib.bo_games_reset_dev(self.h, int(n), slots_ptr, pos_ptr, int(capacity), first_ptr, ply_ptr, stream))

    def search_begin_dev(self, want_ptr: int, nn_in_ptr: int, stream: int = 0):
        self._check(self.lib.bo_search_begin_dev(self.h, want_ptr, nn_in_ptr, stream))

    def analysis_result(self, played_ptr: int, out_ptr: int, stream: int = 0):
        self._check(self.lib.bo_analysis_result(self.h, played_ptr or None, out_ptr, stream))

    def reanalysis_result(self, played_action_ptr: int, root_ptr: int, old_ptr_ptr: int, old_idx_ptr: int, old_val_ptr: int, W: int,
                          out_ptr: int, pi_idx_ptr: int, pi_val_ptr: int, stream: int = 0):
        self._check(self.lib.bo_reanalysis_result(self.h, played_action_ptr or None, root_ptr or None, old_ptr_ptr or None, old_idx_ptr or None,
                                                  old_val_ptr or None, int(W), out_ptr, pi_idx_ptr, pi_val_ptr, stream))

    def root_info(self, stream: int = 0):
        nl, tm, ply = (np.zeros(self.G, dtype=np.int32) for _ in range(3))
        self._check(self.lib.bo_root_info(self.h, _p(nl), _p(tm), _p(ply), stream))
        return nl, tm, ply

    def match_select(self, net_of_white_ptr: int, sel_ptr: int, stream: int = 0):
        self._check(self.lib.bo_match_select(self.h, net_of_white_ptr, sel_ptr, stream))

    def search_begin(self, go, noise: Optional[np.ndarray], nn_in_ptr: int, stream: int = 0):
        g = _i32(go)
        nz = None
        if noise is not None:
            nz = np.ascontiguousarray(noise, dtype=np.float64).reshape(self.G, MAX_LEGAL)
        self._check(self.lib.bo_search_begin(self.h, _p(g), _p(nz, _F64P) if nz is not None else None, nn_in_ptr, stream))

    def step(self, policy_ptr: int, value_ptr: int, kind: int, nn_in_ptr: int, stream: int = 0):
        self._check(self.lib.bo_step(self.h, policy_ptr, value_ptr, kind, nn_in_ptr, stream))

    def step_heads(self, logits_ptr: int, vpart_ptr: int, b1_ptr: int, w2_ptr: int, b2_ptr: int, rows: int, nn_in_ptr: int, stream: int = 0):
        self._check(self.lib.bo_step_heads(self.h, logits_ptr, vpart_ptr, b1_ptr, w2_ptr, b2_ptr, rows, nn_in_ptr, stream))

    def poll(self, stream: int = 0, want_mask: bool = True):
        run, req = C.c_int32(), C.c_int32()
        mask = np.zeros(self.G, dtype=np.int32) if want_mask else None
        self._check(self.lib.bo_search_poll(self.h, C.byref(run), C.byref(req), _p(mask) if want_mask else None, stream))
        return run.value, req.value, mask

    def search_stop(self, mask=None, stream: int = 0) -> np.ndarray:
        m = _i32(mask) if mask is not None else None
        done = np.zeros(self.G, dtype=np.int32)
        self._check(self.lib.bo_search_stop(self.h, _p(m) if m is not None else None, _p(done), stream))
        return done

    def search_close(self, stream: int = 0) -> None:
        self._check(self.lib.bo_search_close(self.h, stream))

    def result(self, stream: int = 0) -> Dict[str, np.ndarray]:
        G = self.G
        out = dict(n=np.zeros(G, np.int32), idx=np.zeros((G, RES_CAP), np.int32), val=np.zeros((G, RES_CAP), np.float32),
                   best_idx=np.zeros(G, np.int32), best_move=np.zeros(G, np.int32), total=np.zeros(G, np.int32))
        self._check(self.lib.bo_search_result(self.h, _p(out["n"]), _p(out["idx"]), _p(out["val"], _F32P),
                                              _p(out["best_idx"]), _p(out["best_move"]), _p(out["total"]), stream))
        return out

    def play(self, actions, stream: int = 0):
        a = _i32(actions)
        assert a.shape == (self.G,)
        self._check(self.lib.bo_play(self.h, _p(a), stream))

    def rng_seed(self, slot: int, seed: int):
        self._check(self.lib.bo_rng_seed(self.h, slot, seed & 0xFFFFFFFF))

    def rng_get_state(self, slot: int):
        key = np.zeros(624, dtype=np.uint32)
        pos, hg, g = C.c_int32(), C.c_int32(), C.c_double()
        self._check(self.lib.bo_rng_state(self.h, slot, 0, key.ctypes.data_as(C.POINTER(C.c_uint32)), C.byref(pos),
                                          C.byref(hg), C.byref(g)))
        return ("MT19937", key, pos.value, hg.value, g.value)

    def rng_set_state(self, slot: int, state):
        key = np.ascontiguousarray(state[1], dtype=np.uint32)
        pos, hg, g = C.c_int32(int(state[2])), C.c_int32(int(state[3])), C.c_double(float(state[4]))
        self._check(self.lib.bo_rng_state(self.h, slot, 1, key.ctypes.data_as(C.POINTER(C.c_uint32)), C.byref(pos),
                                          C.byref(hg), C.byref(g)))

    def selfplay_sample(self, active, move_number, temperature, out, stream: int = 0):
        a, m = _i32(active), _i32(move_number)
        th, ti, tf = temperature
        self._check(self.lib.bo_selfplay_sample(self.h, _p(a), _p(m), int(th), float(ti), float(tf), _p(out["n"]),
                                                _p(out["idx"]), _p(out["val"], _F32P), _p(out["best_idx"]),
                                                _p(out["action"]), stream))
        return out

    def selfplay_noise(self, stream: int = 0):
        self._check(self.lib.bo_selfplay_noise(self.h, stream))

    def selfplay_begun(self):
        nl, tm, go = (np.zeros(self.G, dtype=np.int32) for _ in range(3))
        self._check(self.lib.bo_selfplay_begun(self.h, _p(nl), _p(tm), _p(go)))
        return nl, tm, go

    def result_prefetch(self, stream: int = 0) -> None:
        self._check(self.lib.bo_search_result_prefetch(self.h, stream))

    def selfplay_turn(self, active, move_number, temperature, out, want_next, nn_in_ptr: int, stream: int = 0, defer_noise: bool = False,
                      poll_first: bool = False, lazy_begin: bool = False, prefetched: bool = False):
        a, m, w = _i32(active), _i32(move_number), _i32(want_next)
        th, ti, tf = temperature
        nl, tm, go = (np.zeros(self.G, dtype=np.int32) for _ in range(3))
        done = C.c_int32(0)
        self._check(self.lib.bo_selfplay_turn(self.h, _p(a), _p(m), int(th), float(ti), float(tf), _p(out["n"]), _p(out["idx"]),
                                              _p(out["val"], _F32P), _p(out["best_idx"]), _p(out["action"]), _p(w), nn_in_ptr, _p(nl), _p(tm),
                                              _p(go), (1 if defer_noise else 0) | (2 if poll_first else 0) | (4 if lazy_begin else 0) | (8 if (prefetched and poll_first) else 0),
                                              C.byref(done), stream))
        if done.value < 0:
            return None, None
        if done.value == 2:
            return out, LAZY_BEGIN
        return out, ((nl, tm, go) if done.value else None)

    def selfplay_autoturn(self, active, move_number, temperature, want_next, nn_in_ptr: int, stream: int = 0, redo: bool = False) -> None:
        a, m, w = _i32(active), _i32(move_number), _i32(want_next)
        th, ti, tf = temperature
        self._check(self.lib.bo_selfplay_autoturn(self.h, _p(a), _p(m), int(th), float(ti), float(tf), _p(w), nn_in_ptr, 1 if redo else 0, stream))

    def autoturn_supported(self, temperature) -> bool:
        _, ti, tf = temperature
        if os.environ.get("BETAONE_TURN_COPIES", "0") == "1":
            return False
        return (not self.fast) and int(self.cfg.widen_coeff) == 1 and self.cfg.num_simulations >= 1 and abs(float(ti) - 1.0) < 1e-6 and float(tf) > 0.0

    def autoturn_ready(self) -> bool:
        r = C.c_int32(0)
        self._check(self.lib.bo_selfplay_autoturn_ready(self.h, C.byref(r)))
        return bool(r.value)

    def autoturn_collect(self, out):
        nl, tm, go = (np.zeros(self.G, dtype=np.int32) for _ in range(3))
        done = C.c_int32(0)
        rv, rs = out.get("root_value"), out.get("resigned")
        self._check(self.lib.bo_selfplay_autoturn_collect_ex(self.h, _p(out["n"]), _p(out["idx"]), _p(out["val"], _F32P), _p(out["best_idx"]),
                                                             _p(out["action"]), _p(nl), _p(tm), _p(go),
                                                             _p(rv, _F32P) if rv is not None else None, _p(rs) if rs is not None else None,
                                                             C.byref(done)))
        if done.value < 0:
            return None, None
        return out, (nl, tm, go)

    def root_values(self, on: bool = True) -> None:
        self._check(self.lib.bo_engine_root_values(self.h, 1 if on else 0))

    def selfplay_resign(self, enable, threshold: float, plies: int = 1) -> None:
        e = _i32(enable) if enable is not None else None
        self._check(self.lib.bo_selfplay_resign(self.h, _p(e) if e is not None else None, float(threshold), int(plies)))

    def search_root_value(self, stream: int = 0) -> np.ndarray:
        out = np.zeros(self.G, dtype=np.float32)
        self._check(self.lib.bo_search_root_value(self.h, _p(out, _F32P), stream))
        return out

    def selfplay_begin(self, want, nn_in_ptr: int, stream: int = 0):
        w = _i32(want)
        nl, tm, go = (np.zeros(self.G, dtype=np.int32) for _ in range(3))
        self._check(self.lib.bo_selfplay_begin(self.h, _p(w), nn_in_ptr, _p(nl), _p(tm), _p(go), stream))
        return nl, tm, go

    def export_game(self, slot: int, stream: int = 0, n_plies: Optional[int] = None):
        cap = (self.cfg.max_plies if n_plies is None else min(int(n_plies), self.cfg.max_plies)) + 1
        pos = (BoPosition * cap)()
        mv = np.zeros(cap, dtype=np.int32)
        n = C.c_int32()
        self._check(self.lib.bo_game_export(self.h, slot, pos, _p(mv), cap, C.byref(n), stream))
        return PositionList(pos, n.value + 1), mv[:n.value].tolist()

    def encode_game(self, slot: int, first: int, n: int, out_ptr: int, stream: int = 0):
        self._check(self.lib.bo_game_encode(self.h, slot, first, n, out_ptr, stream))

    def debug_tree(self, slot: int, stream: int = 0) -> List[dict]:
        n = C.c_int32()
        self._check(self.lib.bo_debug_tree(self.h, slot, None, 0, C.byref(n), stream))
        arr = (BoNode * max(1, n.value))()
        self._check(self.lib.bo_debug_tree(self.h, slot, arr, n.value, C.byref(n), stream))
        return [dict(parent=a.parent, n=a.n_visits, q=np.float32(a.q_value), prior=np.float32(a.prior), move=a.move,
                     n_children=a.n_children, first_child=a.first_child, terminal=a.terminal) for a in arr[:n.value]]

    def debug_search_state(self, stream: int = 0) -> Dict[str, np.ndarray]:
        out = np.zeros((5, self.G), np.int32)
        self._check(self.lib.bo_debug_search_state(self.h, _p(out), stream))
        return dict(zip(("phase", "sims_done", "rows", "req_node", "n_nodes"), out))

    def status(self, stream: int = 0) -> Dict[str, np.ndarray]:
        names = ["status", "evals", "flushes", "term_sims", "levels", "children_scanned"]
        out = {k: np.zeros(self.G, np.int32) for k in names}
        self._check(self.lib.bo_engine_status(self.h, *[_p(out[k]) for k in names], stream))
        return out

    TB_SEARCH, TB_ADJUDICATE = 1, 2

    def tablebases(self, tables: Sequence = (), flags: int = 0):
        tables = list(tables)
        arr = (C.c_void_p * max(1, len(tables)))(*[t.h for t in tables])
        rc = self.lib.bo_engine_tablebases(self.h, arr, len(tables), int(flags))
        if rc != 0:
            msg = f"bo_engine_tablebases: {self.lib.bo_last_error().decode()}"
            raise (ValueError if rc in (-1, -3) else EngineError)(msg)
        self._tables = tables

    def tb_stats(self, stream: int = 0) -> Dict[str, np.ndarray]:
        out = {k: np.zeros(self.G, np.int32) for k in ("tb_nodes", "tb_sims", "adjudicated")}
        self._check(self.lib.bo_engine_tb_stats(self.h, _p(out["tb_nodes"]), _p(out["tb_sims"]), _p(out["adjudicated"]), stream))
        return out

    def fast_options(self, tree_reuse=None, games_per_halfwave=None, select_flags=None):
        self._check(self.lib.bo_fast_options(self.h, -1 if tree_reuse is None else (1 if tree_reuse else 0),
                                             -1 if games_per_halfwave is None else int(games_per_halfwave),
                                             -1 if select_flags is None else int(select_flags)))

    SEL_NT, SEL_ROOT_IN_REGS, SEL_DENSE, SEL_LANE, SEL_OCT, SEL_QUAD = 1, 2, 4, 8, 16, 32
    def debug_fast(self, slot: int, stream: int = 0):
        L = self.L
        cs = (16 + 7 * L + 31) // 32 * 32
        ctl, paths = np.zeros(cs, np.int32), np.zeros((L, 64), np.int32)
        self._check(self.lib.bo_debug_fast(self.h, slot, _p(ctl), cs, _p(paths), stream))
        names = ["row_slot", "row_plink", "row_nlegal", "row_term", "row_sim", "sim_row", "sim_plen"]
        out = dict(n_rows=int(ctl[0]), n_step=int(ctl[1]), cur=int(ctl[2]), top=int(ctl[3]), levels=int(ctl[4]), kids=int(ctl[5]),
                   granules=int(ctl[6]), path_nodes=int(ctl[7]), term_sims=int(ctl[8]))
        for i, nm in enumerate(names):
            out[nm] = ctl[16 + i * L:16 + (i + 1) * L].copy()
        return out, paths

    GRANULE_BYTES = 128

    def fast_stats(self, stream: int = 0, time_select: int = -1) -> Dict[str, np.ndarray]:
        gran, pnodes, top = np.zeros(self.G, np.uint64), np.zeros(self.G, np.uint64), np.zeros(self.G, np.int32)
        ms, n = C.c_double(0.0), C.c_int64(0)
        u64 = C.POINTER(C.c_uint64)
        self._check(self.lib.bo_fast_stats(self.h, gran.ctypes.data_as(u64), pnodes.ctypes.data_as(u64), _p(top), time_select,
                                           C.byref(ms), C.byref(n), stream))
        return dict(granules_read=gran, path_nodes=pnodes, arena_granules=top, select_ms=ms.value, select_launches=n.value)

    def event_pair_overhead_ms(self, samples: int = 32, stream: int = 0) -> float:
        ms = C.c_double(0.0)
# ... 44 lines not shown
```

### betaone_amd/rollout.py

```python
from __future__ import annotations

import math
import os
import time
from dataclasses import dataclass, field
from typing import Callable, Dict, List, Optional, Sequence

import numpy as np
import torch

from . import engine as E
from . import sampling

CAPTURE_MODE = "thread_local"


@dataclass
class GameState:
    game_id: int
    rng: object
    start_fen: Optional[str] = None
    start_fullmove: int = 1
    start_white: bool = True
    plies: int = 0
# ... 123 lines not shown
        Rollout._n_instances += 1
        self.tower_timing = torch.zeros(2 + 2 * 4096, dtype=torch.int64, device=self.device) if time_tower else None
        self.G = int(n_games)
        self.S, self.B = int(num_simulations), int(mcts_batch_size)
        self.alpha = float(dirichlet_alpha)
        self.max_game_moves = int(max_game_moves)
        if max_plies is None:
            max_plies = min(self.max_game_moves, 16384) + 2
        self.temperature = temperature
        self.model = model
        self.autocast = autocast
        self.pair = bool(getattr(model, "is_pair", False))
        if self.pair and (fast or autocast):
            raise ValueError("Rollout: a two-net (match) evaluate stage supports the reference search semantics only (fast=False, autocast=False)")
        dev_index = self.device.index if self.device.index is not None else 0
        self.eng = E.Engine(self.G, num_simulations=self.S, mcts_batch_size=self.B, cpuct=cpuct, widen_coeff=widen_coeff,
                            dirichlet_alpha=dirichlet_alpha, dirichlet_epsilon=dirichlet_epsilon, max_plies=max_plies,
                            device=dev_index, fast=fast, leaves_per_step=leaves_per_step, fast_arena_granules=fast_arena_granules)
        self.fast, self.L = bool(fast), self.eng.L
        if self.values:
            self.eng.root_values(True)
        if self.tb is not None:
            self.eng.tablebases(list(self.tb.tables.values()), self.tb_flags)
        self.nn_in = torch.zeros((self.G * self.L, E.INPUT_CHANNELS, 8, 8), dtype=torch.float32, device=self.device)
        self.expected_evals = math.ceil(self.S / self.L) if self.fast else 1 + math.ceil(self.S / self.B)
        self.games: List[Optional[GameState]] = [None] * self.G
        self.use_graph = bool(use_graph) and self.device.type == "cuda"
        self.close_last_eval = self.close_allowed and self.use_graph
        self._graph = None
        self._graphs_n = {}
        self._logits = self._value = None
        self.n_forward = 0
        self.n_sims = 0
        self.n_plies = 0
        self.host_seconds = 0.0
        assert rng_mode in ("python", "native")
        self.rng_mode = rng_mode
        assert policy_kind in ("logits", "probs")
        self.policy_kind = E.POLICY_LOGITS if policy_kind == "logits" else E.POLICY_PROBS
        G = self.G
        self._fgraph = None
        self._side = torch.cuda.Stream(self.device) if self.device.type == "cuda" else None
        self._noise_pending = False
        self._fwd_early = False
        import os as _os
        self.ply_profile = [] if _os.environ.get("BO_PLY_PROFILE", "0") not in ("", "0") else None
        self._t_ret = None
        self._begun = None
        self._turn_due = None
        self._ply_event = None
        self._prefetched = False
        self._auto = False
        self.device_turn = os.environ.get("BETAONE_DEVICE_TURN", "1") != "0"
        self._begun_want = None
        self._active = np.zeros(G, dtype=bool)
        self._plies = np.zeros(G, dtype=np.int64)
        self._start_full = np.ones(G, dtype=np.int64)
        self._start_black = np.zeros(G, dtype=np.int64)
        self._start_step = np.zeros(G, dtype=np.int64)
        self._first_ply = np.zeros(G, dtype=np.int64)
        self._step = 0
        self._hist = {}
        self._pk = 0 if self.fast else 2
        self._pi_n = np.zeros((G, 256), np.int32)
        self._pi_idx = np.zeros((G, 256, max(1, self._pk)), np.int32)
        self._pi_val = np.zeros((G, 256, max(1, self._pk)), np.float32)
        self._out = dict(n=np.zeros(G, np.int32), idx=np.zeros((G, E.RES_CAP), np.int32), val=np.zeros((G, E.RES_CAP), np.float32),
                         best_idx=np.zeros(G, np.int32), action=np.zeros(G, np.int32))
        if self.values:
            self._out.update(root_value=np.zeros(G, np.float32), resigned=np.zeros(G, np.int32))
        self._rv = np.zeros((G, 256 if self.values else 0), np.float32)
        self._resigned = np.zeros(G, dtype=bool)
        self._renable = np.zeros(G, dtype=np.int32)
        self._rcheck = np.zeros(G, dtype=bool)
        self._rcnt = np.zeros((G, 2), dtype=np.int64)
        self.net_of_white = torch.zeros(G, dtype=torch.int32, device=self.device) if self.pair else None
        self._sel = torch.zeros(G, dtype=torch.int32, device=self.device) if self.pair else None
        self._watch_net()
        self._set_tail()

    def _set_tail(self):
        m = self.model
        ok = (self.policy_kind == E.POLICY_LOGITS and not self.fast and not self.autocast and self.device.type == "cuda"
              and os.environ.get("BETAONE_STEP_TAIL", "1") != "0" and hasattr(m, "forward_tail") and m.tail_supported(self.G))
        self.step_tail = bool(ok)
        self._tail_params = tuple(m.tail_params()) if ok else None

    def _step_after(self, first, second):
        if self.step_tail:
            self.eng.step_heads(first.data_ptr(), second.data_ptr(), *self._tail_params, second.shape[1], self.nn_in.data_ptr(), self._stream())
        else:
            self.eng.step(first.data_ptr(), second.data_ptr(), self.policy_kind, self.nn_in.data_ptr(), self._stream())

    def _watch_net(self):
        inner = getattr(self.model, "net", self.model)
        words = getattr(inner, "overflow_words", None)
        self._watch_msg = getattr(inner, "OVERFLOW_MESSAGE", "the evaluate stage reported a fault")
        ptr, n = words() if words is not None else (0, 1)
        self.eng.watch(ptr, n)

    def _check_watch(self):
        if self.eng.watch_seen():
            chk = getattr(getattr(self.model, "net", self.model), "check_overflow", None)
            if chk is not None and self.device.type == "cuda":
                torch.cuda.synchronize(self.device)
                chk()
# ... 15 lines not shown
            if self.step_tail:
                logits, part = self.model.forward_tail(self.nn_in)
                return logits, part
            if fused is not None:
                logits, value = fused(self.nn_in)
                want_probs = False
            elif self.autocast:
                with torch.autocast(self.device.type):
                    logits, value = self.model(self.nn_in)
            else:
                logits, value = self.model(self.nn_in)
        logits = logits.float()
        if want_probs:
            logits = torch.softmax(logits, dim=1)
        return logits.contiguous(), value.float().contiguous()

    def _eval_and_step_eager(self):
        self._stamp(1)
        logits, value = self._forward()
        self._stamp(2)
        self._logits, self._value = logits, value
        self._step_after(logits, value)
        self._stamp(3)

    def _capture(self):
        side = torch.cuda.Stream(self.device)
        side.wait_stream(torch.cuda.current_stream(self.device))
        with torch.cuda.stream(side):
            for _ in range(2):
                self._forward()
        torch.cuda.current_stream(self.device).wait_stream(side)
        torch.cuda.synchronize(self.device)
        g = torch.cuda.CUDAGraph()
        with torch.cuda.graph(g, capture_error_mode=CAPTURE_MODE):
            logits, value = self._forward()
            self._step_after(logits, value)
        self._graph, self._logits, self._value = g, logits, value

    def _eval_and_step(self):
        self.n_forward += 1
        if self.use_graph:
            if self._graph is None:
                self._capture()
            self._graph.replay()
        else:
            self._eval_and_step_eager()

    MAX_GRAPH_ITERATIONS = 12

    def _eval_and_step_n(self, n: int, close: Optional[bool] = None):
        if close is None:
            close = self.close_last_eval
        close = bool(close) and n >= 2
        iters = n - 1 if close else n
        if n <= 1 or not self.use_graph:
            for _ in range(iters):
                self._eval_and_step()
            if close:
                self.eng.search_close(self._stream())
            return
        if n > self.MAX_GRAPH_ITERATIONS:
            while n > 0:
                k = min(n, self.MAX_GRAPH_ITERATIONS)
                self._eval_and_step_n(k, close and k == n)
                n -= k
            return
        key = (n, True) if close else n
        g = self._graphs_n.get(key)
        if g is None:
            if self._graph is None:
                self._capture()
            cg, keep = torch.cuda.CUDAGraph(), []
            with torch.cuda.graph(cg, capture_error_mode=CAPTURE_MODE):
                for _ in range(iters):
                    self._stamp(1)
                    logits, value = self._forward()
                    self._stamp(2)
                    self._step_after(logits, value)
                    self._stamp(3)
                    keep.append((logits, value))
                if close:
                    self.eng.search_close(self._stream())
            g = self._graphs_n[key] = (cg, keep)
        self.n_forward += iters
        g[0].replay()

    @_on_main
    def start_games(self, slots: Sequence[int], game_ids: Sequence[int], rngs: Sequence, fens: Optional[Sequence] = None,
                    moves: Optional[Sequence] = None, net_of_white: Optional[Sequence[int]] = None):
        self._start_games(slots, game_ids, rngs, fens, moves, net_of_white)

    def _start_games(self, slots, game_ids, rngs, fens=None, moves=None, net_of_white=None):
        if self.pair:
            if net_of_white is None or len(net_of_white) != len(slots) or any(v not in (0, 1) for v in net_of_white):
                raise ValueError("Rollout.start_games: a two-net evaluate stage needs net_of_white (0 / 1) for every game")
            self.net_of_white[torch.as_tensor(list(slots), dtype=torch.long, device=self.device)] = \
                torch.as_tensor(list(net_of_white), dtype=torch.int32).to(self.device)
        self.eng.reset(list(slots), fens, moves, stream=self._stream())
        for i, s in enumerate(slots):
            fen = fens[i] if fens is not None else None
            full, white = _fen_meta(fen)
            self.games[s] = GameState(game_id=int(game_ids[i]), rng=rngs[i], start_fen=fen, start_fullmove=full,
                                      start_white=white)
            if moves is not None and moves[i]:
                self.games[s].plies = self.games[s].first_ply = len(moves[i].split())
            self._active[s] = True
            if self._begun_want is not None:
                self._begun_want[s] = False
            self._plies[s] = self._first_ply[s] = self.games[s].plies
            self._start_full[s], self._start_black[s] = full, 0 if white else 1
            self._start_step[s] = self._step
            self._resigned[s] = False
            self._rcnt[s] = 0
            self._rcheck[s] = self.resign and resign_check_game(game_ids[i], self.resign_f)
            self._renable[s] = 1 if (self.resign and not self._rcheck[s]) else 0
            if self.rng_mode == "native":
                self.eng.rng_seed(s, int(rngs[i]))

    @_on_main
    def search(self, go: np.ndarray, n_legal: np.ndarray, terminal: np.ndarray) -> Dict[str, np.ndarray]:
        t0 = time.perf_counter()
        noise = None
        if self.alpha > 0:
            noise = np.zeros((self.G, E.MAX_LEGAL), dtype=np.float64)
            for g in np.nonzero(go)[0]:
                if terminal[g] == 0:
                    noise[g, :n_legal[g]] = sampling.root_noise(n_legal[g], self.alpha, self.games[g].rng)
        self.host_seconds += time.perf_counter() - t0
        stream = self._stream()
        self.eng.search_begin(go, noise, self.nn_in.data_ptr(), stream)
        self.eng.step(0, 0, E.POLICY_NONE, self.nn_in.data_ptr(), stream)
        burst = self.expected_evals
        while True:
            for _ in range(burst):
                self._eval_and_step()
            running, _, _ = self.eng.poll(self._stream(), want_mask=False)
            if running == 0:
                break
# ... 64 lines not shown

    def _resign_decide(self, go, rv, plies) -> np.ndarray:
        out = np.zeros(self.G, dtype=bool)
        if not self.resign:
            return out
        for g in np.nonzero(np.asarray(go, bool) & (self._renable != 0))[0]:
            par = int(plies[g]) & 1
            c = self._rcnt[g, par] + 1 if np.float32(rv[g]) < self.resign_t else 0
            self._rcnt[g, par] = c
            out[g] = c >= self.resign_k
        return out

    def _forward_only(self):
        if not self.use_graph:
            self._f_logits, self._f_value = self._forward()
            return
        if self._fgraph is None:
            if self._graph is None:
                self._capture()
            g = torch.cuda.CUDAGraph()
            with torch.cuda.graph(g, capture_error_mode=CAPTURE_MODE):
                logits, value = self._forward()
            self._fgraph, self._f_logits, self._f_value = g, logits, value
        self._fgraph.replay()

    PLY_TRACE = []

    def _pp(self, name):
        now = time.perf_counter()
        self.ply_profile.append((name, now - self._pp_t))
        if os.environ.get("BO_PLY_PROFILE") == "trace":
            Rollout.PLY_TRACE.append((self._pp_t, now, self._stamp_id, name))
        self._pp_t = now

    def _run_search_steps(self, poll: bool = True):
        burst = self.expected_evals
        info = None
        if self._noise_pending:
            self._noise_pending = False
            if self._fwd_early:
                self._fwd_early = False
            else:
                self.n_forward += 1
                self._forward_only()
            if self._begun is E.LAZY_BEGIN:
                info = self.eng.selfplay_begun()
                self._begun = None
            if self.ply_profile is not None: self._pp("begun")
            self.eng.selfplay_noise(self._stream())
            if self.ply_profile is not None: self._pp("noise")
            self._step_after(self._f_logits, self._f_value)
            burst -= 1
        while True:
            self._eval_and_step_n(burst)
            if not poll:
                return info
            running, _, _ = self.eng.poll(self._stream(), want_mask=False)
            if running == 0:
                break
            burst = 1

    def _play_ply_native(self, on_finished, refill, while_searching=None) -> int:
        if self._turn_due is not None:
            self.ply_end()
        if not self.ply_begin(on_finished, refill, while_searching):
            return 0
        return self.ply_end()

    @_on_main
    def ply_begin(self, on_finished=None, refill=None, while_searching=None) -> bool:
        assert self.rng_mode == "native" and self._turn_due is None
        eng, G = self.eng, self.G
        stream = self._stream()
        t0 = time.perf_counter()
        if self.ply_profile is not None:
            if self._t_ret is not None:
                self.ply_profile.append(("between_calls", t0 - self._t_ret))
            self._pp_t = t0
        want = self._active & (self._plies < self.max_game_moves)
        limit_done = np.nonzero(self._active & ~want)[0]
        resign_done = np.nonzero(want & self._resigned)[0]
        want &= ~self._resigned
        self.host_seconds += time.perf_counter() - t0
        lazy = False
        if self._begun is not None:
            extra = want & ~self._begun_want
            if self._begun is E.LAZY_BEGIN and not extra.any():
                lazy = True
            else:
                if extra.any():
                    self._fwd_early = False
                nl, term, go = eng.selfplay_begun() if self._begun is E.LAZY_BEGIN else self._begun
                self._begun = None
                if extra.any():
                    nl2, t2, go2 = eng.selfplay_begin(extra.astype(np.int32), self.nn_in.data_ptr(), stream)
                    nl, term, go = np.where(extra, nl2, nl), np.where(extra, t2, term), go | go2
        else:
            nl, term, go = eng.selfplay_begin(want.astype(np.int32), self.nn_in.data_ptr(), stream)
        if lazy:
            nl, term, go = self._run_search_steps(poll=False)
        if self.ply_profile is not None: self._pp("enqueue_search")
        if len(resign_done):
            term = np.array(term, copy=True)
            term[resign_done] = 3
        done = [int(g) for g in limit_done] + [int(g) for g in resign_done] + [int(g) for g in np.nonzero(want & (term != 0))[0]]
        for g in done:
            self._active[g] = False
        if not go.any():
            self._fwd_early = False
            self._noise_pending = False
            self._finish_and_refill(done, term, on_finished, refill)
            if while_searching is not None:
                while_searching()
            return False
        if not lazy:
            self._run_search_steps(poll=False)
        if done:
            if self._side is not None:
                with torch.cuda.stream(self._side):
                    self._finish_and_refill(done, term, on_finished, refill)
            else:
                self._finish_and_refill(done, term, on_finished, refill)
        if self.ply_profile is not None: self._pp("finish_and_refill")
        if while_searching is not None:
            while_searching()
        if self.ply_profile is not None: self._pp("while_searching")
        self._turn_due = go
        if self._device_turn_ok():
            self._enqueue_autoturn(go)
        else:
            self._prefetch_result()
        self._mark_enqueued()
        if self.ply_profile is not None: self._pp("enqueue_turn")
        return True

    def _device_turn_ok(self) -> bool:
        return self.device_turn and self.eng.autoturn_supported(self.temperature)

    def _enqueue_autoturn(self, go: np.ndarray, redo: bool = False) -> None:
        move_number = self._start_full + (self._plies + self._start_black) // 2
        want_next = self._active & ((self._plies + go) < self.max_game_moves)
        self._auto_want = want_next
        if self.resign:
            self.eng.selfplay_resign(self._renable, float(self.resign_t), self.resign_k)
        self.eng.selfplay_autoturn(go, move_number, self.temperature, want_next.astype(np.int32), self.nn_in.data_ptr(), self._stream(), redo=redo)
        self._auto = True
        self._prefetched = False
        if want_next.any():
            self.n_forward += 1
            self._forward_only()
            self._fwd_early = True

    PREFETCH_RESULT = os.environ.get("BETAONE_RESULT_PREFETCH", "1") != "0"

    def _prefetch_result(self) -> None:
        self._prefetched = False
        if self.PREFETCH_RESULT and not self.fast:
            self.eng.result_prefetch(self._stream())
            self._prefetched = True

    def _mark_enqueued(self) -> None:
        if self.device.type == "cuda":
            if self._ply_event is None:
                self._ply_event = torch.cuda.Event()
            self._ply_event.record(torch.cuda.current_stream(self.device))

    def ply_ready(self) -> bool:
        if self._turn_due is not None and self._auto:
            return self.eng.autoturn_ready()
        return self._turn_due is not None and (self._ply_event is None or self._ply_event.query())

    @_on_main
    def ply_end(self, block: bool = True, drop: Sequence[int] = ()) -> Optional[int]:
        eng, G = self.eng, self.G
        stream = self._stream()
        go, self._turn_due = self._turn_due, None
        if len(drop):
            go = go.copy()
            go[list(drop)] = 0
        t0 = time.perf_counter()
        if self.ply_profile is not None: self._pp_t = t0
        move_number = self._start_full + (self._plies + self._start_black) // 2
        want_next = self._active & ((self._plies + go) < self.max_game_moves)
        self.host_seconds += time.perf_counter() - t0
        out = None
        if self._auto:
            want_next = self._auto_want
            while True:
                out, begun = eng.autoturn_collect(self._out)
                if out is not None:
                    self._auto = False
                    break
                self._fwd_early = False
                if self.ply_profile is not None: self.ply_profile.append(("redo_turn", 0.0))
                self._check_watch()
                self._eval_and_step()
                self._enqueue_autoturn(go, redo=True)
                if not block:
# ... 379 lines not shown
```

### include/betaone_engine.h

```cpp
#ifndef BETAONE_ENGINE_H
#define BETAONE_ENGINE_H

#include <stdint.h>

#ifdef __cplusplus
extern "C" {
#endif

#define BO_ABI_VERSION 18
#define BO_NUM_ACTIONS 4672
#define BO_INPUT_CHANNELS 120
#define BO_ROW_FLOATS (120 * 64)
#define BO_MAX_LEGAL 256
#define BO_RES_CAP 256

enum {
    BO_OK = 0,
    BO_E_ARG = -1,
    BO_E_HIP = -2,
    BO_E_CONFIG = -3,
    BO_E_FEN = -4,
    BO_E_STATE = -5
};

enum {
    BO_ST_NODE_OVERFLOW = 1, BO_ST_DEPTH_OVERFLOW = 2, BO_ST_NAN_SCORE = 4, BO_ST_PLY_OVERFLOW = 8,
    BO_ST_ILLEGAL_ACTION = 16, BO_ST_UL_OVERFLOW = 32, BO_ST_TRK_OVERFLOW = 64,
    BO_ST_BAD_RANGE = 128,
    BO_ST_PI_OVERFLOW = 256
};

enum { BO_POLICY_NONE = 0, BO_POLICY_LOGITS = 1, BO_POLICY_PROBS = 2 };

typedef struct {
    int32_t n_games;
    int32_t num_simulations;
    int32_t mcts_batch_size;
    int32_t max_plies;
    double cpuct;
    double widen_coeff;
    double dirichlet_alpha;
    double dirichlet_epsilon;
    int32_t mode;
    int32_t leaves_per_step;
    int32_t fast_arena_granules;
} bo_config;

typedef struct {
    uint64_t bb[8];
    int32_t turn;
    uint32_t castling;
    int32_t ep_square;
    int32_t ep_key;
    int32_t halfmove_clock;
    int32_t fullmove_number;
} bo_position;

typedef struct bo_engine bo_engine;

int bo_abi_version(void);
const char *bo_last_error(void);

int bo_engine_create(const bo_config *cfg, int device, bo_engine **out);
void bo_engine_destroy(bo_engine *e);

int bo_games_reset(bo_engine *e, int n, const int32_t *slots, const char *const *fens, const char *const *moves,
                   void *stream);

int bo_games_reset_ex(bo_engine *e, int n, const int32_t *slots, const char *const *fens, const char *const *moves,
                      const bo_position *hist, const int32_t *n_hist, const bo_position *trk,
                      const int32_t *trk_counts, const int32_t *trk_off, void *stream);

int bo_root_info(bo_engine *e, int32_t *n_legal, int32_t *terminal, int32_t *ply, void *stream);

int bo_search_begin(bo_engine *e, const int32_t *go, const double *noise, float *nn_in_dev, void *stream);

int bo_step(bo_engine *e, const float *policy_dev, const float *value_dev, int policy_kind, float *nn_in_dev,
            void *stream);
int bo_step_heads(bo_engine *e, const float *logits_dev, const float *vpart_dev, const float *b1_dev, const float *w2_dev,
                  const float *b2_dev, int rows, float *nn_in_dev, void *stream);

int bo_search_poll(bo_engine *e, int32_t *n_running, int32_t *n_requested, int32_t *requested_mask, void *stream);

int bo_search_stop(bo_engine *e, const int32_t *stop_mask, int32_t *sims_done, void *stream);

int bo_search_close(bo_engine *e, void *stream);

int bo_search_result(bo_engine *e, int32_t *res_n, int32_t *res_idx, float *res_val, int32_t *best_idx,
                     int32_t *best_move, int32_t *total_visits, void *stream);

int bo_play(bo_engine *e, const int32_t *action, void *stream);

int bo_rng_seed(bo_engine *e, int slot, uint32_t seed);
int bo_rng_state(bo_engine *e, int slot, int set, uint32_t *key624, int32_t *pos, int32_t *has_gauss, double *gauss);
int bo_selfplay_sample(bo_engine *e, const int32_t *active, const int32_t *move_number, int32_t threshold,
                       double t_initial, double t_final, int32_t *res_n, int32_t *res_idx, float *res_val,
                       int32_t *best_idx, int32_t *action_out, void *stream);
int bo_selfplay_begin(bo_engine *e, const int32_t *want, float *nn_in_dev, int32_t *n_legal_out, int32_t *terminal_out,
                      int32_t *go_out, void *stream);

int bo_selfplay_turn(bo_engine *e, const int32_t *active, const int32_t *move_number, int32_t threshold, double t_initial,
                     double t_final, int32_t *res_n, int32_t *res_idx, float *res_val, int32_t *best_idx, int32_t *action_out,
                     const int32_t *want_next, float *nn_in_dev, int32_t *n_legal_out, int32_t *terminal_out, int32_t *go_out,
                     int32_t defer_noise, int32_t *completed, void *stream);
int bo_selfplay_begun(bo_engine *e, int32_t *n_legal_out, int32_t *terminal_out, int32_t *go_out);
int bo_search_result_prefetch(bo_engine *e, void *stream);
int bo_selfplay_noise(bo_engine *e, void *stream);

int bo_selfplay_autoturn(bo_engine *e, const int32_t *active, const int32_t *move_number, int32_t threshold, double t_initial,
                         double t_final, const int32_t *want_next, float *nn_in_dev, int32_t redo, void *stream);
int bo_selfplay_autoturn_ready(bo_engine *e, int32_t *ready_out);
int bo_selfplay_autoturn_collect(bo_engine *e, int32_t *res_n, int32_t *res_idx, float *res_val, int32_t *best_idx, int32_t *action_out,
                                 int32_t *n_legal_out, int32_t *terminal_out, int32_t *go_out, int32_t *completed);

int bo_selfplay_autoturn_collect_ex(bo_engine *e, int32_t *res_n, int32_t *res_idx, float *res_val, int32_t *best_idx, int32_t *action_out,
                                    int32_t *n_legal_out, int32_t *terminal_out, int32_t *go_out, float *root_value_out,
                                    int32_t *resigned_out, int32_t *completed);
int bo_engine_root_values(bo_engine *e, int32_t on);
int bo_selfplay_resign(bo_engine *e, const int32_t *enable, float threshold, int32_t plies);
int bo_search_root_value(bo_engine *e, float *out, void *stream);

int bo_game_export(bo_engine *e, int slot, bo_position *positions, int32_t *moves, int32_t cap, int32_t *n_plies,
                   void *stream);
int bo_game_encode(bo_engine *e, int slot, int first, int n, float *out_dev, void *stream);

int bo_records_encode(int n_positions, const bo_position *positions, int first, int n, float *out_dev, void *stream);

int bo_fast_options(bo_engine *e, int32_t tree_reuse, int32_t games_per_halfwave, int32_t select_flags);
#define BO_FAST_GRANULE_BYTES 128
int bo_engine_status(bo_engine *e, int32_t *status, int32_t *evals, int32_t *flushes, int32_t *term_sims,
                     int32_t *levels, int32_t *children_scanned, void *stream);


int bo_movegen_batch(bo_engine *e, int n, const bo_position *pos, int32_t *moves_out, int32_t *n_out,
                     int32_t *check_out, void *stream);


int bo_nn_bias_act(float *x_dev, const float *bias_dev, const float *residual_dev, int batch, int channels, void *stream);
int bo_nn_se_residual(float *x_dev, const float *bias_dev, const float *w1_dev, const float *w2_dev,
                      const float *residual_dev, int batch, int channels, int hidden, void *stream);

int bo_nn_se_residual_small(const float *x_dev, const float *bias_dev, const float *w1_dev, const float *w2_dev,
                            float *residual_inout_dev, int batch, int channels, int hidden, void *stream);
int bo_nn_heads(const void *p_dev, const void *v_dev, const float *wp_dev, const float *bp_dev, const float *w1_dev,
                const float *b1_dev, const float *w2_dev, const float *b2_dev, float *policy_out_dev, float *value_out_dev,
                float *scratch_dev, int batch, int flags, void *stream);
int bo_nn_heads_f16(const void *p_dev, const void *v_dev, const void *wp_f16_dev, const float *bp_dev, const void *w1_f16_dev,
                    const float *b1_dev, const float *w2_dev, const float *b2_dev, float *policy_out_dev, float *value_out_dev,
                    float *scratch_dev, int batch, int flags, void *stream);
int bo_nn_conv3x3(const float *x_dev, const float *wpacked_dev, const float *bias_dev, const float *residual_dev,
                  float *y_dev, int batch, int c_in, int c_out, int mode, void *stream);

int bo_nn_conv3x3_small(const float *x_dev, const float *wpacked_dev, const float *bias_dev, const float *residual_dev, float *y_dev,
                        int batch, int c_in, int c_in_x, int c_out, int mode, void *stream);

enum { BO_TOWER_DIRECT = 0, BO_TOWER_WINOGRAD = 1, BO_TOWER_DIRECT_F16 = 2, BO_TOWER_SPLIT_F16 = 3, BO_TOWER_SPLIT_F16_T16 = 4, BO_TOWER_DIRECT_F16_T16 = 5 };
typedef struct bo_tower_layer_desc {
    int32_t w_off4, t4, bias_off, kind, se_w1_off, se_w2_off, hidden, last;
} bo_tower_layer_desc;
typedef struct bo_tower_head_desc {
    int32_t channels, split, w_off, b_off;
} bo_tower_head_desc;
typedef struct bo_tower_s bo_tower;
// ... 247 lines not shown
```

### include/betaone_lab.h

```cpp
#ifndef BETAONE_LAB_H
#define BETAONE_LAB_H

#include "betaone_engine.h"

#ifdef __cplusplus
extern "C" {
#endif

#define BO_PROF_SLOTS 16

typedef struct {
    int32_t parent, n_visits, first_child, n_children;
    float q_value, prior;
    int32_t move;
    int32_t terminal;
} bo_node;
int bo_debug_tree(bo_engine *e, int slot, bo_node *out, int32_t cap, int32_t *n_nodes, void *stream);
int bo_debug_search_state(bo_engine *e, int32_t *out, void *stream);

int bo_fast_stats(bo_engine *e, uint64_t *granules_read, uint64_t *path_nodes, int32_t *arena_granules, int32_t time_select, double *select_ms,
                  int64_t *select_launches, void *stream);

int bo_event_pair_overhead(double *ms_out, int32_t samples, void *stream);

int bo_debug_fast(bo_engine *e, int slot, int32_t *ctl_out, int32_t ctl_cap, int32_t *paths_out, void *stream);

int bo_debug_profile(bo_engine *e, int enable, uint64_t *cycles_out, void *stream);

int bo_select_wide(const void *blocks_dev, const int32_t *root_block_dev, const int32_t *root_n_dev,
                   const float *sqrt_lut_dev, int n_trees, int max_depth, float cpuct, int grid_blocks,
                   int32_t *out_leaf_dev, int32_t *out_levels_dev, void *stream);

int bo_nn_tower_forward_timed(bo_tower *tower, const float *x_dev, float *y_dev, void *head_a_dev, void *head_b_dev, int batch,
                              void *timing_dev, void *stream);

int bo_debug_stamp(void *ring_dev, uint64_t tag, uint64_t capacity, void *stream);

int bo_nn_b1_profile(bo_b1 *tower, int enable, uint64_t *out, int cap);

#ifdef __cplusplus
}
#endif
#endif
```

Before: 80.70 million.

## Fuse search close, turn sampling, play and begin into fewer launches

```diff
diff --git a/betaone_amd/csrc/bo_engine.cpp b/betaone_amd/csrc/bo_engine.cpp
--- a/betaone_amd/csrc/bo_engine.cpp
+++ b/betaone_amd/csrc/bo_engine.cpp
@@ -63,6 +63,7 @@
     bo_config cfg;
     int device;
     std::vector<void *> allocs;
+    std::vector<size_t> alloc_bytes;
     int *d_go = nullptr, *d_action = nullptr;
     std::vector<int> h_i32;
     std::vector<HostRng> rng;
@@ -106,6 +107,7 @@
         int rc = rt_malloc(&v, n * sizeof(T));
         if (rc) return rc;
         allocs.push_back(v);
+        alloc_bytes.push_back(n * sizeof(T));
         *p = (T *)v;
         return 0;
     }
@@ -282,7 +284,9 @@
     rc |= e->alloc(&d.prof, G * BO_PROF_SLOTS);
     rc |= e->alloc(&d.resign_cnt, 2 * G); rc |= e->alloc(&e->d_root_value, G);
     if (!rc) rt_memset(d.resign_cnt, 0, 2 * G * 4, nullptr);
-    rc |= e->alloc(&e->d_tb_tabs, (size_t)TB_MAX_TABLES); rc |= e->alloc(&d.tb_stat, 3 * G);
+    rc |= e->alloc(&e->d_tb_tabs, (size_t)TB_MAX_TABLES);
+    if (!rc) e->alloc_bytes.back() = 0;
+    rc |= e->alloc(&d.tb_stat, 3 * G);
     if (!rc) rt_memset(d.tb_stat, 0, 3 * G * 4, nullptr);
     d.tb_tabs = e->d_tb_tabs; d.tb_n = 0; d.tb_flags = 0;
     d.played_now = nullptr;
@@ -538,7 +542,7 @@
 #undef SEL
 }
 
-static int step_launch(bo_engine *e, const float *policy_dev, const float *value_dev, int policy_kind, float *nn_in_dev, void *stream, const StepTail &vt) {
+static int step_launch(bo_engine *e, const float *policy_dev, const float *value_dev, int policy_kind, float *nn_in_dev, void *stream, const StepTail *vt) {
     e->prefetch_valid = false;
     if (e->fast) {
         const int rows = e->d.c.G * e->f.L;
@@ -561,8 +565,12 @@
 #endif
         RT(RT_LAUNCH(bo_k_fw_leaf, rows, stream, e->d, e->f, nn_in_dev));
     } else {
-        if (e->d.tb_n > 0 && (e->d.tb_flags & TBF_SEARCH)) RT(RT_LAUNCH(bo_k_step_tb, e->d.c.G, stream, e->d, policy_dev, value_dev, policy_kind, nn_in_dev, vt));
-        else RT(RT_LAUNCH(bo_k_step, e->d.c.G, stream, e->d, policy_dev, value_dev, policy_kind, nn_in_dev, vt));
+        const bool tb = e->d.tb_n > 0 && (e->d.tb_flags & TBF_SEARCH);
+        if (vt) {
+            if (tb) RT(RT_LAUNCH(bo_k_step_tb_tail, e->d.c.G, stream, e->d, policy_dev, value_dev, policy_kind, nn_in_dev, *vt));
+            else RT(RT_LAUNCH(bo_k_step_tail, e->d.c.G, stream, e->d, policy_dev, value_dev, policy_kind, nn_in_dev, *vt));
+        } else if (tb) RT(RT_LAUNCH(bo_k_step_tb, e->d.c.G, stream, e->d, policy_dev, value_dev, policy_kind, nn_in_dev));
+        else RT(RT_LAUNCH(bo_k_step, e->d.c.G, stream, e->d, policy_dev, value_dev, policy_kind, nn_in_dev));
     }
     return BO_OK;
 }
@@ -570,14 +578,15 @@
                        void *stream) {
     if (!e || !nn_in_dev) return fail(BO_E_ARG, "null argument");
     if (policy_kind != BO_POLICY_NONE && (!policy_dev || !value_dev)) return fail(BO_E_ARG, "policy/value required");
-    return step_launch(e, policy_dev, value_dev, policy_kind, nn_in_dev, stream, StepTail{nullptr, nullptr, nullptr, nullptr, 0});
+    return step_launch(e, policy_dev, value_dev, policy_kind, nn_in_dev, stream, nullptr);
 }
 extern "C" int bo_step_heads(bo_engine *e, const float *logits_dev, const float *vpart_dev, const float *b1_dev, const float *w2_dev,
                              const float *b2_dev, int rows, float *nn_in_dev, void *stream) {
     if (!e || !nn_in_dev || !logits_dev || !vpart_dev || !b1_dev || !w2_dev || !b2_dev) return fail(BO_E_ARG, "null argument");
     if (e->fast) return fail(BO_E_CONFIG, "bo_step_heads: the reference-semantics search only (fast mode evaluates rows, not games)");
     if (rows < e->d.c.G) return fail(BO_E_ARG, "bo_step_heads: the partial sums must hold a row per game (rows >= G)");
-    return step_launch(e, logits_dev, nullptr, BO_POLICY_LOGITS, nn_in_dev, stream, StepTail{vpart_dev, b1_dev, w2_dev, b2_dev, rows});
+    const StepTail vt{vpart_dev, b1_dev, w2_dev, b2_dev, rows};
+    return step_launch(e, logits_dev, nullptr, BO_POLICY_LOGITS, nn_in_dev, stream, &vt);
 }
 
 extern "C" int bo_search_poll(bo_engine *e, int32_t *n_running, int32_t *n_requested, int32_t *requested_mask, void *stream) {
@@ -949,8 +958,8 @@
     return BO_OK;
 }
 
-extern "C" int bo_selfplay_autoturn(bo_engine *e, const int32_t *active, const int32_t *move_number, int32_t threshold, double t_initial,
-                                    double t_final, const int32_t *want_next, float *nn_in_dev, int32_t redo, void *stream) {
+static int autoturn_impl(bo_engine *e, const int32_t *active, const int32_t *move_number, int32_t threshold, double t_initial,
+                         double t_final, const int32_t *want_next, float *nn_in_dev, int32_t redo, bool fused, int32_t close, void *stream) {
     if (!e || !active || !move_number || !want_next || !nn_in_dev) return fail(BO_E_ARG, "null argument");
     if (e->fast || e->d.c.root_m != 1 || e->d.c.S < 1)
         return fail(BO_E_CONFIG, "bo_selfplay_autoturn: reference-semantics engines whose root keeps <= 2 children (int(WIDEN_COEFF) == 1, NUM_SIMULATIONS >= 1)");
@@ -990,17 +999,34 @@
     a.resign_t = e->resign_t; a.resign_k = e->resign_k;
     e->prefetch_valid = false;
     e->nl_valid = false;
-    RT(RT_LAUNCH(bo_k_turn_sample, G, stream, e->d, a));
-    RT(RT_LAUNCH(bo_k_turn_play, G, stream, e->d, a, nn_in_dev));
     const size_t Gs = (size_t)G, watch_off = Gs * (4 + 2 * (size_t)BO_RES_CAP);
-    int rc = ship(e, e->h_info + 2 * Gs, (const int *)e->d_info_blk + 2 * Gs, 15 * Gs, e->h_res + watch_off, (const int *)e->d_res_blk + watch_off, 4, stream);
-    if (rc) return rc;
+    int rc;
+    if (fused) {
+        if (close && e->d.c.root_q) return fail(BO_E_STATE, "bo_selfplay_autoturn_fused: close with root values on (a closed search's q values lack the last evaluation)");
+        RT(RT_LAUNCH(bo_k_turn_close_sample, G, stream, e->d, a, close ? 1 : 0));
+        RT(RT_LAUNCH(bo_k_turn_play_begin, G, stream, e->d, a, nn_in_dev, (TurnOut{e->h_info, e->h_res + watch_off, (const int *)e->d_res_blk + watch_off})));
+    } else {
+        RT(RT_LAUNCH(bo_k_turn_sample, G, stream, e->d, a));
+        RT(RT_LAUNCH(bo_k_turn_play, G, stream, e->d, a, nn_in_dev));
+        rc = ship(e, e->h_info + 2 * Gs, (const int *)e->d_info_blk + 2 * Gs, 15 * Gs, e->h_res + watch_off, (const int *)e->d_res_blk + watch_off, 4, stream);
+        if (rc) return rc;
+    }
     if (!e->ev_turn_made) { RT(rt_event_create(&e->ev_turn)); e->ev_turn_made = true; }
     RT(rt_event_record(e->ev_turn, stream));
-    rc = bo_step(e, nullptr, nullptr, BO_POLICY_NONE, nn_in_dev, stream);
-    if (rc) return rc;
+    if (!fused || redo) {
+        rc = bo_step(e, nullptr, nullptr, BO_POLICY_NONE, nn_in_dev, stream);
+        if (rc) return rc;
+    }
     e->turn_outstanding = true;
     return BO_OK;
+}
+extern "C" int bo_selfplay_autoturn(bo_engine *e, const int32_t *active, const int32_t *move_number, int32_t threshold, double t_initial,
+                                    double t_final, const int32_t *want_next, float *nn_in_dev, int32_t redo, void *stream) {
+    return autoturn_impl(e, active, move_number, threshold, t_initial, t_final, want_next, nn_in_dev, redo, false, 0, stream);
+}
+extern "C" int bo_selfplay_autoturn_fused(bo_engine *e, const int32_t *active, const int32_t *move_number, int32_t threshold, double t_initial,
+                                          double t_final, const int32_t *want_next, float *nn_in_dev, int32_t redo, int32_t close, void *stream) {
+    return autoturn_impl(e, active, move_number, threshold, t_initial, t_final, want_next, nn_in_dev, redo, true, close, stream);
 }
 
 extern "C" int bo_selfplay_autoturn_ready(bo_engine *e, int32_t *ready_out) {
@@ -2041,6 +2067,26 @@
     if (!ok) return fail(BO_E_CONFIG, "bo_train_metrics: unsupported dtype");
     if (!rc) rc = RT_LAUNCH(bo_k_metrics_reduce, n_buckets, stream, (int)n, (const float *)rows_dev, (const int *)bucket_dev, accum_dev);
     if (rc) return fail(BO_E_HIP, std::string("bo_train_metrics: ") + rt_errstr(rc));
+    return BO_OK;
+}
+
+extern "C" int bo_debug_state_dump(bo_engine *e, uint8_t *out, int64_t cap, int64_t *need_out, void *stream) {
+    if (!e || !need_out) return fail(BO_E_ARG, "bad arguments");
+    const size_t G = (size_t)e->d.c.G, res_bytes = (G * (4 + 2 * (size_t)BO_RES_CAP) + 4) * 4, info_bytes = G * 18 * 4;
+    size_t need = res_bytes + info_bytes;
+    for (size_t b : e->alloc_bytes) need += b;
+    *need_out = (int64_t)need;
+    if (!out) return BO_OK;
+    if (cap < (int64_t)need) return fail(BO_E_ARG, "bo_debug_state_dump: buffer too small");
+    RT(rt_sync(stream));
+    size_t off = 0;
+    for (size_t i = 0; i < e->allocs.size(); i++) {
+        if (e->alloc_bytes[i]) RT(rt_d2h(out + off, e->allocs[i], e->alloc_bytes[i], stream));
+        off += e->alloc_bytes[i];
+    }
+    RT(rt_sync(stream));
+    memcpy(out + off, e->h_info, info_bytes);
+    memcpy(out + off + info_bytes, e->h_res, res_bytes);
     return BO_OK;
 }
 
diff --git a/betaone_amd/csrc/bo_tree.h b/betaone_amd/csrc/bo_tree.h
--- a/betaone_amd/csrc/bo_tree.h
+++ b/betaone_amd/csrc/bo_tree.h
@@ -362,7 +362,7 @@
 }
 template <bool TB>
 BO_DEV int terminal_burst(const Eng &e, int g, const int *path, int d, float v, int sims_left, float *lds, bool *staged,
-                          const int *pb = nullptr, int db = 0, float vb = 0.0f, int *n_swaps = nullptr) {
+                          const int *pb, int db, float vb, int &n_swaps) {
     const bool lone = TB && db < 0;
     const size_t no = NOFF(e, g);
     const int lane = bo_lane(), grp = lane >> 4, j = lane & 15;
@@ -513,7 +513,7 @@
             { const float t_ = v_cur; v_cur = v_oth; v_oth = t_; }
             last_l = grp == d - 1;
             last_bits = 0xFFFFull << (16 * (d - 1));
-            if (n_swaps) *n_swaps += 1;
+            n_swaps += 1;
             continue;
         }
         if ((mb & last_bits) != 0) {
@@ -769,7 +769,8 @@
     return tanhf(((s[0] + s[1]) + (s[2] + s[3])) + r.b2);
 }
 
-BO_DEV void apply_leaf(const Eng &e, int g, int leaf, const float *row, int kind, const float *value_of, const StepTail &vt, StepShared &sh,
+template <bool TAIL>
+BO_DEV void apply_leaf(const Eng &e, int g, int leaf, const float *row, int kind, const float *value_of, StepTail vt, StepShared &sh,
                        int *n_ul_io, int *flags) {
     const size_t no = NOFF(e, g);
     const int lane = bo_lane();
@@ -784,7 +785,7 @@
         for (int j = lane; j < n; j += 64) sh.pv[j] = row[move_to_index(mv[j])];
     } else {
         float mx, sum;
-        if (vt.vpart) {
+        if constexpr (TAIL) {
             TailRegs tr;
             tail_load(vt, g, tr);
             row_max_sum(row, &mx, &sum);
@@ -816,8 +817,8 @@
     const float m = 1.0f - (float)kc * (1.0f / 1024.0f);
     return t == TERM_TB_LOSS ? m : t == TERM_TB_WIN ? -m : 0.0f;
 }
-template <bool TB>
-BO_DEV int step_body(const Eng &e, int g, const float *policy, const float *value, int kind, float *nn_in, StepShared &sh, const StepTail &vt) {
+template <bool TB, bool TAIL>
+BO_DEV int step_body(const Eng &e, int g, const float *policy, const float *value, int kind, float *nn_in, StepShared &sh, StepTail vt) {
     const int lane = bo_lane();
     const size_t no = NOFF(e, g);
     int flags = 0;
@@ -837,7 +838,7 @@
     const float *lut = e.sqrt_lut;
     if (req >= 0) {
         if (req == 0) apply_root(e, g, policy + (size_t)g * BO_NUM_ACTIONS, kind, sh, &n_nodes, &flags);
-        else apply_leaf(e, g, req, policy + (size_t)g * BO_NUM_ACTIONS, kind, value, vt, sh, &n_ul, &flags);
+        else apply_leaf<TAIL>(e, g, req, policy + (size_t)g * BO_NUM_ACTIONS, kind, value, vt, sh, &n_ul, &flags);
         req = -1;
     }
     BO_PROF(0)
@@ -902,7 +903,7 @@
             if (small) {
                 const bool small_b = b_depth > 0 && e.c.burst_two != 0;
                 applied = terminal_burst<TB>(e, g, sh.path, depth, tv, may, sh.probs, &burst_tables_staged, sh.bpath, tb_leaf ? -1 : small_b ? b_depth : 0, b_tv,
-                                             &n_swaps);
+                                             n_swaps);
                 n_burst++; n_burst_sims += applied;
                 bo_sync();
                 if (lane <= depth) sh.bpath[lane] = sh.path[lane];
@@ -957,17 +958,29 @@
     }
     return n_nodes;
 }
-BO_KERNEL void bo_k_step(Eng e, const float *policy, const float *value, int kind, float *nn_in, StepTail vt) {
+BO_KERNEL void bo_k_step(Eng e, const float *policy, const float *value, int kind, float *nn_in) {
     BO_SHARED StepShared sh;
     const int g = bo_block();
     if (e.phase[g] != PH_RUN) return;
-    step_body<false>(e, g, policy, value, kind, nn_in, sh, vt);
-}
-BO_KERNEL void bo_k_step_tb(Eng e, const float *policy, const float *value, int kind, float *nn_in, StepTail vt) {
+    step_body<false, false>(e, g, policy, value, kind, nn_in, sh, StepTail{nullptr, nullptr, nullptr, nullptr, 0});
+}
+BO_KERNEL void bo_k_step_tb(Eng e, const float *policy, const float *value, int kind, float *nn_in) {
     BO_SHARED StepShared sh;
     const int g = bo_block();
     if (e.phase[g] != PH_RUN) return;
-    step_body<true>(e, g, policy, value, kind, nn_in, sh, vt);
+    step_body<true, false>(e, g, policy, value, kind, nn_in, sh, StepTail{nullptr, nullptr, nullptr, nullptr, 0});
+}
+BO_KERNEL void bo_k_step_tail(Eng e, const float *policy, const float *value, int kind, float *nn_in, StepTail vt) {
+    BO_SHARED StepShared sh;
+    const int g = bo_block();
+    if (e.phase[g] != PH_RUN) return;
+    step_body<false, true>(e, g, policy, value, kind, nn_in, sh, vt);
+}
+BO_KERNEL void bo_k_step_tb_tail(Eng e, const float *policy, const float *value, int kind, float *nn_in, StepTail vt) {
+    BO_SHARED StepShared sh;
+    const int g = bo_block();
+    if (e.phase[g] != PH_RUN) return;
+    step_body<true, true>(e, g, policy, value, kind, nn_in, sh, vt);
 }
 
 BO_DEV int root_prepare(const Eng &e, int g, StepShared &sh) {
@@ -1096,8 +1109,8 @@
     }
 }
 
-BO_KERNEL void bo_k_search_close(Eng e) {
-    const int g = bo_block(), lane = bo_lane();
+BO_DEV void close_body(const Eng &e, int g) {
+    const int lane = bo_lane();
     if (e.phase[g] != PH_RUN) return;
     const size_t no = NOFF(e, g);
     const int req = e.req_node[g], n_nodes = e.n_nodes[g];
@@ -1118,6 +1131,7 @@
         if (flags) e.status[g] |= flags;
     }
 }
+BO_KERNEL void bo_k_search_close(Eng e) { close_body(e, bo_block()); }
 
 BO_KERNEL void bo_k_ship(int *dst_a, const int *src_a, int n_a, int *dst_b, const int *src_b, int n_b, int n_blocks) {
     const int i0 = bo_block() * 64 + bo_lane(), stride = n_blocks * 64;
@@ -1250,8 +1264,8 @@
     return (k0 / last > u) ? i0 : i1;
 }
 
-BO_KERNEL void bo_k_turn_sample(Eng e, TurnArgs a) {
-    const int g = bo_block(), lane = bo_lane();
+BO_DEV void turn_sample_body(const Eng &e, const TurnArgs &a, int g) {
+    const int lane = bo_lane();
     result_body(e, g);
     const int fl = a.flags[g], ph = e.phase[g];
     int st = 0, act = -1, n = 0, ia = -1, ib = -1, ca = 0, cb = 0, total = 0, rsg = 0, rnext = -1;
@@ -1287,20 +1301,54 @@
         c[7] = n >= 2 ? __builtin_bit_cast(int, (float)((double)cb / (double)total)) : 0;
     }
 }
-
+BO_KERNEL void bo_k_turn_sample(Eng e, TurnArgs a) { turn_sample_body(e, a, bo_block()); }
+BO_KERNEL void bo_k_turn_close_sample(Eng e, TurnArgs a, int close) {
+    const int g = bo_block();
+    if (close) { close_body(e, g); bo_sync(); }
+    turn_sample_body(e, a, g);
+}
+
+BO_DEV bool turn_play_body(const Eng &e, const TurnArgs &a, float *nn_in, int g, StepShared &sh) {
+    const int lane = bo_lane();
+    if (lane == 0 && a.resign_next[g] >= 0) e.resign_cnt[2 * g + (e.ply[g] & 1)] = a.resign_next[g];
+    if (a.resigned[g]) return false;
+    int t = play_body(e, g, a.action[g], sh);
+    if (t < 0) t = e.root_term[g];
+    if (!(a.flags[g] & 4) || t != 0) return false;
+    encode_static(e, g, nn_in + (size_t)g * BO_ROW);
+    if (lane == 0) e.phase[g] = PH_RUN;
+    return true;
+}
+BO_DEV bool turn_any_bad(const Eng &e, const TurnArgs &a) {
+    const int lane = bo_lane();
+    bool bad = false;
+    for (int j0 = 0; j0 < e.c.G; j0 += 64) bad = bad || bo_ballot(j0 + lane < e.c.G && a.state[j0 + lane] != 0) != 0;
+    return bad;
+}
 BO_KERNEL void bo_k_turn_play(Eng e, TurnArgs a, float *nn_in) {
     BO_SHARED StepShared sh;
+    if (turn_any_bad(e, a)) return;
+    turn_play_body(e, a, nn_in, bo_block(), sh);
+}
+
+struct TurnOut { int *info; int *watch; const int *d_watch; };
+BO_KERNEL void bo_k_turn_play_begin(Eng e, TurnArgs a, float *nn_in, TurnOut o) {
+    BO_SHARED StepShared sh;
     const int g = bo_block(), lane = bo_lane();
-    bool bad = false;
-    for (int j0 = 0; j0 < e.c.G; j0 += 64) bad = bad || bo_ballot(j0 + lane < e.c.G && a.state[j0 + lane] != 0) != 0;
-    if (bad) return;
-    if (lane == 0 && a.resign_next[g] >= 0) e.resign_cnt[2 * g + (e.ply[g] & 1)] = a.resign_next[g];
-    if (a.resigned[g]) return;
-    int t = play_body(e, g, a.action[g], sh);
-    if (t < 0) t = e.root_term[g];
-    if (!(a.flags[g] & 4) || t != 0) return;
-    encode_static(e, g, nn_in + (size_t)g * BO_ROW);
-    if (lane == 0) e.phase[g] = PH_RUN;
+    const size_t G = (size_t)e.c.G;
+    if (!turn_any_bad(e, a)) {
+        const bool begun = turn_play_body(e, a, nn_in, g, sh);
+        bo_sync();
+        if (begun) step_body<false, false>(e, g, nn_in, nn_in, POLICY_NONE, nn_in, sh, StepTail{nullptr, nullptr, nullptr, nullptr, 0});
+        bo_sync();
+    }
+    if (lane == 0) {
+        o.info[2 * G + g] = e.root_nlegal[g]; o.info[3 * G + g] = e.root_term[g]; o.info[4 * G + g] = e.ply[g];
+        o.info[5 * G + g] = a.action[g]; o.info[6 * G + g] = a.state[g];
+        o.info[15 * G + g] = __builtin_bit_cast(int, a.root_value[g]); o.info[16 * G + g] = a.resigned[g];
+    }
+    if (lane < 8) o.info[7 * G + (size_t)g * 8 + lane] = a.cres[(size_t)g * 8 + lane];
+    if (g == 0 && lane < 4) o.watch[lane] = o.d_watch[lane];
 }
 
 BO_KERNEL void bo_k_root_value(Eng e, float *out) {
diff --git a/betaone_amd/engine.py b/betaone_amd/engine.py
--- a/betaone_amd/engine.py
+++ b/betaone_amd/engine.py
@@ -107,6 +107,7 @@
                                    C.c_void_p, _I32P, _I32P, _I32P, C.c_int32, _I32P, C.c_void_p]),
     "bo_selfplay_noise": (C.c_int, [C.c_void_p, C.c_void_p]),
     "bo_selfplay_autoturn": (C.c_int, [C.c_void_p, _I32P, _I32P, C.c_int32, C.c_double, C.c_double, _I32P, C.c_void_p, C.c_int32, C.c_void_p]),
+    "bo_selfplay_autoturn_fused": (C.c_int, [C.c_void_p, _I32P, _I32P, C.c_int32, C.c_double, C.c_double, _I32P, C.c_void_p, C.c_int32, C.c_int32, C.c_void_p]),
     "bo_selfplay_autoturn_ready": (C.c_int, [C.c_void_p, _I32P]),
     "bo_selfplay_autoturn_collect": (C.c_int, [C.c_void_p, _I32P, _I32P, _F32P, _I32P, _I32P, _I32P, _I32P, _I32P, _I32P]),
     "bo_selfplay_autoturn_collect_ex": (C.c_int, [C.c_void_p, _I32P, _I32P, _F32P, _I32P, _I32P, _I32P, _I32P, _I32P, _F32P, _I32P, _I32P]),
@@ -217,6 +218,7 @@
 _LAB_SYMBOLS = {
     "bo_debug_tree": (C.c_int, [C.c_void_p, C.c_int, C.POINTER(BoNode), C.c_int32, _I32P, C.c_void_p]),
     "bo_debug_search_state": (C.c_int, [C.c_void_p, _I32P, C.c_void_p]),
+    "bo_debug_state_dump": (C.c_int, [C.c_void_p, C.c_void_p, C.c_int64, C.POINTER(C.c_int64), C.c_void_p]),
     "bo_debug_fast": (C.c_int, [C.c_void_p, C.c_int, _I32P, C.c_int32, _I32P, C.c_void_p]),
     "bo_event_pair_overhead": (C.c_int, [_F64P, C.c_int32, C.c_void_p]),
     "bo_nn_b1_profile": (C.c_int, [C.c_void_p, C.c_int, C.POINTER(C.c_uint64), C.c_int]),
@@ -241,7 +243,7 @@
 
 
 _hip_lib: Optional[C.CDLL] = None
-ABI_VERSION = 18
+ABI_VERSION = 19
 PROF_SLOTS = 16
 METRIC_ROW = {name: k for k, name in enumerate((
     "BAD", "HAS_POLICY", "DECISIVE", "RANK", "TOP1", "TOP3", "TOP5", "ARGMAX_IN_SUPPORT", "CE", "TARGET_ENTROPY", "NET_ENTROPY", "P_TOP",
@@ -359,6 +361,8 @@
         h = C.c_void_p()
         self._check(self.lib.bo_engine_create(C.byref(self.cfg), device, C.byref(h)))
         self.h = h
+        self.close_in_turn = False
+        self.close_due = False
 
     def close(self):
         if getattr(self, "h", None):
@@ -458,6 +462,9 @@
         return done
 
     def search_close(self, stream: int = 0) -> None:
+        if self.close_in_turn:
+            self.close_due = True
+            return
         self._check(self.lib.bo_search_close(self.h, stream))
 
     def result(self, stream: int = 0) -> Dict[str, np.ndarray]:
@@ -524,9 +531,17 @@
             return out, LAZY_BEGIN
         return out, ((nl, tm, go) if done.value else None)
 
-    def selfplay_autoturn(self, active, move_number, temperature, want_next, nn_in_ptr: int, stream: int = 0, redo: bool = False) -> None:
+    def selfplay_autoturn(self, active, move_number, temperature, want_next, nn_in_ptr: int, stream: int = 0, redo: bool = False,
+                          fused: bool = False) -> None:
+        close, self.close_due = self.close_due and not redo, False
+        if close and not fused:
+            self._check(self.lib.bo_search_close(self.h, stream))
         a, m, w = _i32(active), _i32(move_number), _i32(want_next)
         th, ti, tf = temperature
+        if fused:
+            self._check(self.lib.bo_selfplay_autoturn_fused(self.h, _p(a), _p(m), int(th), float(ti), float(tf), _p(w), nn_in_ptr, 1 if redo else 0,
+                                                            1 if close else 0, stream))
+            return
         self._check(self.lib.bo_selfplay_autoturn(self.h, _p(a), _p(m), int(th), float(ti), float(tf), _p(w), nn_in_ptr, 1 if redo else 0, stream))
 
     def autoturn_supported(self, temperature) -> bool:
@@ -593,6 +608,13 @@
         out = np.zeros((5, self.G), np.int32)
         self._check(self.lib.bo_debug_search_state(self.h, _p(out), stream))
         return dict(zip(("phase", "sims_done", "rows", "req_node", "n_nodes"), out))
+
+    def debug_state_dump(self, stream: int = 0) -> np.ndarray:
+        need = C.c_int64()
+        self._check(self.lib.bo_debug_state_dump(self.h, None, 0, C.byref(need), stream))
+        out = np.zeros(need.value, np.uint8)
+        self._check(self.lib.bo_debug_state_dump(self.h, out.ctypes.data, need.value, C.byref(need), stream))
+        return out
 
     def status(self, stream: int = 0) -> Dict[str, np.ndarray]:
         names = ["status", "evals", "flushes", "term_sims", "levels", "children_scanned"]
diff --git a/betaone_amd/rollout.py b/betaone_amd/rollout.py
--- a/betaone_amd/rollout.py
+++ b/betaone_amd/rollout.py
@@ -199,6 +199,8 @@
         self._prefetched = False
         self._auto = False
         self.device_turn = os.environ.get("BETAONE_DEVICE_TURN", "1") != "0"
+        self.turn_fused = os.environ.get("BETAONE_TURN_FUSED", "1") != "0"
+        self._defer_close = False
         self._begun_want = None
         self._active = np.zeros(G, dtype=bool)
         self._plies = np.zeros(G, dtype=np.int64)
@@ -320,12 +322,13 @@
         if close is None:
             close = self.close_last_eval
         close = bool(close) and n >= 2
+        defer = close and self._defer_close
         iters = n - 1 if close else n
         if n <= 1 or not self.use_graph:
             for _ in range(iters):
                 self._eval_and_step()
             if close:
-                self.eng.search_close(self._stream())
+                self._search_close(defer)
             return
         if n > self.MAX_GRAPH_ITERATIONS:
             while n > 0:
@@ -335,7 +338,7 @@
             return
         key = (n, True) if close else n
         g = self._graphs_n.get(key)
-        if g is None:
+        if g is None or g[2] != defer:
             if self._graph is None:
                 self._capture()
             cg, keep = torch.cuda.CUDAGraph(), []
@@ -347,11 +350,20 @@
                     self._step_after(logits, value)
                     self._stamp(3)
                     keep.append((logits, value))
-                if close:
+                if close and not defer:
                     self.eng.search_close(self._stream())
-            g = self._graphs_n[key] = (cg, keep)
+            g = self._graphs_n[key] = (cg, keep, defer)
         self.n_forward += iters
         g[0].replay()
+        if defer:
+            self._search_close(True)
+
+    def _search_close(self, defer: bool):
+        self.eng.close_in_turn = bool(defer)
+        try:
+            self.eng.search_close(self._stream())
+        finally:
+            self.eng.close_in_turn = False
 
     @_on_main
     def start_games(self, slots: Sequence[int], game_ids: Sequence[int], rngs: Sequence, fens: Optional[Sequence] = None,
@@ -522,7 +534,11 @@
             self._step_after(self._f_logits, self._f_value)
             burst -= 1
         while True:
-            self._eval_and_step_n(burst)
+            self._defer_close = not poll and self.turn_fused and self._device_turn_ok()
+            try:
+                self._eval_and_step_n(burst)
+            finally:
+                self._defer_close = False
             if not poll:
                 return info
             running, _, _ = self.eng.poll(self._stream(), want_mask=False)
@@ -579,6 +595,7 @@
         if not go.any():
             self._fwd_early = False
             self._noise_pending = False
+            self.eng.close_due = False
             self._finish_and_refill(done, term, on_finished, refill)
             if while_searching is not None:
                 while_searching()
@@ -613,7 +630,8 @@
         self._auto_want = want_next
         if self.resign:
             self.eng.selfplay_resign(self._renable, float(self.resign_t), self.resign_k)
-        self.eng.selfplay_autoturn(go, move_number, self.temperature, want_next.astype(np.int32), self.nn_in.data_ptr(), self._stream(), redo=redo)
+        self.eng.selfplay_autoturn(go, move_number, self.temperature, want_next.astype(np.int32), self.nn_in.data_ptr(), self._stream(), redo=redo,
+                                   fused=self.turn_fused)
         self._auto = True
         self._prefetched = False
         if want_next.any():
diff --git a/include/betaone_engine.h b/include/betaone_engine.h
--- a/include/betaone_engine.h
+++ b/include/betaone_engine.h
@@ -7,7 +7,7 @@
 extern "C" {
 #endif
 
-#define BO_ABI_VERSION 18
+#define BO_ABI_VERSION 19
 #define BO_NUM_ACTIONS 4672
 #define BO_INPUT_CHANNELS 120
 #define BO_ROW_FLOATS (120 * 64)
@@ -109,6 +109,8 @@
 
 int bo_selfplay_autoturn(bo_engine *e, const int32_t *active, const int32_t *move_number, int32_t threshold, double t_initial,
                          double t_final, const int32_t *want_next, float *nn_in_dev, int32_t redo, void *stream);
+int bo_selfplay_autoturn_fused(bo_engine *e, const int32_t *active, const int32_t *move_number, int32_t threshold, double t_initial,
+                               double t_final, const int32_t *want_next, float *nn_in_dev, int32_t redo, int32_t close, void *stream);
 int bo_selfplay_autoturn_ready(bo_engine *e, int32_t *ready_out);
 int bo_selfplay_autoturn_collect(bo_engine *e, int32_t *res_n, int32_t *res_idx, float *res_val, int32_t *best_idx, int32_t *action_out,
                                  int32_t *n_legal_out, int32_t *terminal_out, int32_t *go_out, int32_t *completed);
diff --git a/include/betaone_lab.h b/include/betaone_lab.h
--- a/include/betaone_lab.h
+++ b/include/betaone_lab.h
@@ -17,6 +17,7 @@
 } bo_node;
 int bo_debug_tree(bo_engine *e, int slot, bo_node *out, int32_t cap, int32_t *n_nodes, void *stream);
 int bo_debug_search_state(bo_engine *e, int32_t *out, void *stream);
+int bo_debug_state_dump(bo_engine *e, uint8_t *out, int64_t cap, int64_t *need_out, void *stream);
 
 int bo_fast_stats(bo_engine *e, uint64_t *granules_read, uint64_t *path_nodes, int32_t *arena_granules, int32_t time_select, double *select_ms,
                   int64_t *select_launches, void *stream);
```

Result: no change. 81.31 million, median of 6 (+0.8%).
